# ronnymilleo/amcpy

Hardware: AMD Instinct MI355X
Metric: IQ frames/sec (18 features, 2048-sample complex64) (higher is better)
Workload: dtype f32; 1 GPU; 6 mods x 26 SNR x 4096 frames x 2048 samples complex64 per GPU (BASELINE configs[1]), resident in HBM; one launch per step; frame_size=2048, kernel=amcx_features18_wave_kernel<2048>

## Files before the change

amcpy_amd/csrc/amcx.hip:

```cpp
#include "../../include/amcx.h"

#include <hip/hip_runtime.h>
#include <stdio.h>
#include <stdlib.h>
#include <string.h>
#include <chrono>
#include <new>

#include "amcx_block_kernel.h"
#include "amcx_stream_kernel.h"
#include "amcx_wave_kernel.h"
#include "amcx_quad_kernel.h"
#include "amcx_group_kernel.h"
#include "amcx_short_kernel.h"
#include "amcx_post_kernels.h"
#include "amcx_pack_kernel.h"
#include "amcx_upload.h"

namespace {

thread_local char g_hip_err[256] = "";

int hip_fail(hipError_t e, const char* what) {
  snprintf(g_hip_err, sizeof g_hip_err, "%s: %s", what, hipGetErrorString(e));
  return AMCX_EHIP;
}

#define AMCX_HIP(call)                                     \
  do {                                                     \
    hipError_t e_ = (call);                                \
    if (e_ != hipSuccess) return hip_fail(e_, #call);      \
  } while (0)

bool is_pow2(int n) { return n > 0 && (n & (n - 1)) == 0; }

int resolve_variant(int32_t frame_size, int32_t variant) {
  if (frame_size < AMCX_MIN_FRAME_SIZE || frame_size > AMCX_MAX_FRAME_SIZE) return AMCX_EINVAL;
  const bool block_ok = frame_size <= AMCX_MAX_BLOCK_FRAME_SIZE;
  switch (variant) {
    case AMCX_VARIANT_AUTO:
      return amcx::wave_supports(frame_size) ? AMCX_VARIANT_WAVE : block_ok ? AMCX_VARIANT_BLOCK : AMCX_ENOTSUP;
    case AMCX_VARIANT_BLOCK:
      return block_ok ? AMCX_VARIANT_BLOCK : AMCX_ENOTSUP;
    case AMCX_VARIANT_WAVE:
      return amcx::wave_supports(frame_size) ? AMCX_VARIANT_WAVE : AMCX_ENOTSUP;
    default:
      return AMCX_EINVAL;
  }
}

int cu_count() {
  static int cus[64] = {};
  int dev = 0, n = 0;
  if (hipGetDevice(&dev) != hipSuccess) { (void)hipGetLastError(); return 256; }
  if (dev >= 0 && dev < 64 && cus[dev] > 0) return cus[dev];
  if (hipDeviceGetAttribute(&n, hipDeviceAttributeMultiprocessorCount, dev) != hipSuccess || n <= 0) {
    (void)hipGetLastError();
    return 256;
  }
  if (dev >= 0 && dev < 64) cus[dev] = n;
  return n;
}

bool on_another_device(const void* p) {
  hipPointerAttribute_t a;
  if (hipPointerGetAttributes(&a, p) != hipSuccess) { (void)hipGetLastError(); return false; }
  if (a.type != hipMemoryTypeDevice) return false;
  int dev = 0;
  if (hipGetDevice(&dev) != hipSuccess) { (void)hipGetLastError(); return false; }
  return a.device != dev;
}

int block_mode(int N) {
  if (is_pow2(N)) return amcx::kBlockPow2;
  if (N >= amcx::kBluesteinMinN && N <= amcx::kBluesteinMaxN) return amcx::kBlockBluestein;
  return N > amcx::kBluesteinMaxN ? amcx::kBlockBluesteinBig : amcx::kBlockDirect;
}

struct StreamPlan {
  int M;
  bool chirped;
  int64_t grid;
};

StreamPlan stream_plan(int32_t N, int64_t n_frames) {
  StreamPlan p;
  p.M = amcx::stream::conv_length(N);
  p.chirped = !is_pow2(N);
  p.grid = cu_count();
  if (p.grid > n_frames) p.grid = n_frames;
  if (p.grid < 1) p.grid = 1;
  return p;
}

int set_stream_lds_once(const void* kern, int which) {
  static bool attr_set[3][64] = {};
  int dev = 0;
  AMCX_HIP(hipGetDevice(&dev));
  if (dev < 0 || dev >= 64 || !attr_set[which][dev]) {
    const size_t most = which == 0 ? amcx::stream::lds_bytes(amcx::stream::kMaxN)
                        : which == 1 ? amcx::stream::lds_bytes_fft(amcx::stream::kMaxN)
                                     : (size_t)amcx::stream::kTileBytes + amcx::stream::kFftTabBytes;
    AMCX_HIP(hipFuncSetAttribute(kern, hipFuncAttributeMaxDynamicSharedMemorySize, (int)most));
    if (dev >= 0 && dev < 64) attr_set[which][dev] = true;
  }
  return AMCX_OK;
}

int launch_stream(const float2* iq, int64_t n_frames, int32_t N, int64_t row_stride, float* out,
                  int64_t out_stride, hipStream_t stream, void* ws, int64_t ws_bytes) {
  StreamPlan p = stream_plan(N, n_frames);
  const int64_t per = (int64_t)p.M * (int64_t)sizeof(float2);
  int64_t fit = ws != nullptr && ws_bytes > 0 ? ws_bytes / per - (p.chirped ? 1 : 0) : 0;
  if (fit >= 1 && (reinterpret_cast<uintptr_t>(ws) & 7u) == 0) {
    if (p.grid > fit) p.grid = fit;
    float2* const base = static_cast<float2*>(ws);
    const float2* bspec = nullptr;
    float2* bufs = base;
    if (p.chirped) {
      auto chirp = amcx::stream::amcx_stream_chirp_kernel;
      const int rc = set_stream_lds_once(reinterpret_cast<const void*>(chirp), 2);
      if (rc != AMCX_OK) return rc;
      hipLaunchKernelGGL(chirp, dim3(1), dim3(amcx::stream::kThreads),
                         (size_t)amcx::stream::kTileBytes + amcx::stream::kFftTabBytes, stream, base, (int)N, p.M);
      AMCX_HIP(hipGetLastError());
      bspec = base;
      bufs = base + p.M;
    }
    auto kern = amcx::stream::amcx_features18_stream_kernel<true>;
    const int rc = set_stream_lds_once(reinterpret_cast<const void*>(kern), 1);
    if (rc != AMCX_OK) return rc;
    hipLaunchKernelGGL(kern, dim3((unsigned)p.grid), dim3(amcx::stream::kThreads), amcx::stream::lds_bytes_fft(N), stream,
                       iq, (long long)n_frames, (int)N, (long long)row_stride, out, (long long)out_stride, bspec, bufs, p.M);
    AMCX_HIP(hipGetLastError());
    return AMCX_OK;
  }
  auto kern = amcx::stream::amcx_features18_stream_kernel<false>;
  const int rc = set_stream_lds_once(reinterpret_cast<const void*>(kern), 0);
  if (rc != AMCX_OK) return rc;
  hipLaunchKernelGGL(kern, dim3((unsigned)p.grid), dim3(amcx::stream::kThreads), amcx::stream::lds_bytes(N), stream, iq,
                     (long long)n_frames, (int)N, (long long)row_stride, out, (long long)out_stride,
                     static_cast<const float2*>(nullptr), static_cast<float2*>(nullptr), 0);
  AMCX_HIP(hipGetLastError());
  return AMCX_OK;
}

int launch_block(const float2* iq, int64_t n_frames, int32_t N, int64_t row_stride, float* out,
                 int64_t out_stride, hipStream_t stream, void* ws = nullptr, int64_t ws_bytes = 0) {
  if (N > amcx::kBlockMaxN) return launch_stream(iq, n_frames, N, row_stride, out, out_stride, stream, ws, ws_bytes);
  const int mode = block_mode(N);
  const size_t lds = (mode == amcx::kBlockBluestein      ? (size_t)16 * amcx::bluestein_length(N)
                      : mode == amcx::kBlockBluesteinBig ? (size_t)8 * amcx::kBluesteinBigM
                                                         : (size_t)16 * N) +
                     amcx::kBlockScratchBytes + amcx::kBlockTwiddleBytes;
  auto kern = mode == amcx::kBlockPow2           ? amcx::amcx_features18_block_kernel<amcx::kBlockPow2>
              : mode == amcx::kBlockBluestein    ? amcx::amcx_features18_block_kernel<amcx::kBlockBluestein>
              : mode == amcx::kBlockBluesteinBig ? amcx::amcx_features18_block_kernel<amcx::kBlockBluesteinBig>
                                                 : amcx::amcx_features18_block_kernel<amcx::kBlockDirect>;
  {
    static bool attr_set[4][64] = {};
    constexpr int kMaxLds = 16 * amcx::kBlockMaxN + amcx::kBlockScratchBytes + amcx::kBlockTwiddleBytes;
    int dev = 0;
    AMCX_HIP(hipGetDevice(&dev));
    if (dev < 0 || dev >= 64 || !attr_set[mode][dev]) {
      AMCX_HIP(hipFuncSetAttribute(reinterpret_cast<const void*>(kern),
                                   hipFuncAttributeMaxDynamicSharedMemorySize, kMaxLds));
      if (dev >= 0 && dev < 64) attr_set[mode][dev] = true;
    }
  }
  const int per_cu = (int)((160 * 1024) / lds) < 1 ? 1 : (int)((160 * 1024) / lds);
  int64_t grid = (int64_t)cu_count() * (per_cu > 8 ? 8 : per_cu) * 4;
  if (grid > n_frames) grid = n_frames;
  hipLaunchKernelGGL(kern, dim3((unsigned)grid), dim3(amcx::kBlockThreads), lds, stream, iq,
                     (long long)n_frames, (int)N, (long long)row_stride, out, (long long)out_stride);
  AMCX_HIP(hipGetLastError());
  return AMCX_OK;
}

__global__ __launch_bounds__(1024) void amcx_probe_fma_kernel(int iters, float* sink, unsigned long long* ticks) {
  float a0 = (float)threadIdx.x, a1 = a0 + 1.f, a2 = a0 + 2.f, a3 = a0 + 3.f, a4 = a0 + 4.f, a5 = a0 + 5.f,
        a6 = a0 + 6.f, a7 = a0 + 7.f;
  const float b0 = 1.0001f, b1 = 0.9999f;
  const unsigned long long t0 = __builtin_amdgcn_s_memtime();
  const unsigned long long r0 = __builtin_amdgcn_s_memrealtime();
  for (int i = 0; i < iters; ++i) {
#pragma unroll
    for (int u = 0; u < 4; ++u)
      asm volatile(
          "v_fma_f32 %0, %0, %8, %9\n v_fma_f32 %1, %1, %8, %9\n v_fma_f32 %2, %2, %8, %9\n v_fma_f32 %3, %3, %8, %9\n"
          "v_fma_f32 %4, %4, %8, %9\n v_fma_f32 %5, %5, %8, %9\n v_fma_f32 %6, %6, %8, %9\n v_fma_f32 %7, %7, %8, %9\n"
          : "+v"(a0), "+v"(a1), "+v"(a2), "+v"(a3), "+v"(a4), "+v"(a5), "+v"(a6), "+v"(a7) : "v"(b0), "v"(b1));
  }
  const unsigned long long t1 = __builtin_amdgcn_s_memtime();
  const unsigned long long r1 = __builtin_amdgcn_s_memrealtime();
  const float s = ((a0 + a1) + (a2 + a3)) + ((a4 + a5) + (a6 + a7));
  if (s == 12345.678f) sink[0] = s;
  if ((threadIdx.x & 63) == 0) {
    const long long w = ((long long)blockIdx.x * blockDim.x + threadIdx.x) >> 6;
    ticks[2 * w] = t1 - t0;
    ticks[2 * w + 1] = r1 - r0;
  }
}

__global__ __launch_bounds__(256) void amcx_probe_read_kernel(const float4* __restrict__ src,
                                                             long long n_vec, float* partial) {
  typedef float v4f __attribute__((ext_vector_type(4)));
  float acc = 0.f;
  const long long stride = (long long)gridDim.x * blockDim.x;
  long long i = (long long)blockIdx.x * blockDim.x + threadIdx.x;
  for (; i + 3 * stride < n_vec; i += 4 * stride) {
    const v4f a = __builtin_nontemporal_load(reinterpret_cast<const v4f*>(src + i));
    const v4f b = __builtin_nontemporal_load(reinterpret_cast<const v4f*>(src + i + stride));
    const v4f c = __builtin_nontemporal_load(reinterpret_cast<const v4f*>(src + i + 2 * stride));
    const v4f d = __builtin_nontemporal_load(reinterpret_cast<const v4f*>(src + i + 3 * stride));
    acc += ((a.x + a.y) + (a.z + a.w)) + ((b.x + b.y) + (b.z + b.w)) + ((c.x + c.y) + (c.z + c.w)) +
           ((d.x + d.y) + (d.z + d.w));
  }
  for (; i < n_vec; i += stride) {
    const float4 v = src[i];
    acc += (v.x + v.y) + (v.z + v.w);
  }
#pragma unroll
  for (int off = 32; off >= 1; off >>= 1) acc += __shfl_xor(acc, off, 64);
  __shared__ float s[4];
  if ((threadIdx.x & 63) == 0) s[threadIdx.x >> 6] = acc;
  __syncthreads();
  if (threadIdx.x == 0) partial[blockIdx.x] = (s[0] + s[1]) + (s[2] + s[3]);
}

}

extern "C" {

int amcx_abi_version(void) { return AMCX_ABI_VERSION; }

const char* amcx_strerror(int code) {
  switch (code) {
    case AMCX_OK: return "ok";
    case AMCX_EINVAL: return "invalid argument (null pointer, negative count, stride or frame_size out of range)";
    case AMCX_ENOTSUP: return "kernel variant does not support this frame_size";
    case AMCX_EHIP: return "HIP runtime error (see amcx_last_hip_error)";
    case AMCX_ENODEV: return "no usable gfx950 device";
    case AMCX_ENOMEM: return "device memory allocation failed";
    case AMCX_EIO: return "reading the container's file failed (see amcx_last_hip_error for the errno text)";
    default: return "unknown amcx error code";
  }
}

const char* amcx_last_hip_error(void) { return g_hip_err; }

int amcx_device_count(void) {
  int n = 0;
  hipError_t e = hipGetDeviceCount(&n);
  if (e == hipErrorNoDevice) return 0;
  if (e != hipSuccess) return hip_fail(e, "hipGetDeviceCount");
  int ok = 0;
  for (int d = 0; d < n; ++d) {
    hipDeviceProp_t p;
    if (hipGetDeviceProperties(&p, d) == hipSuccess && strncmp(p.gcnArchName, "gfx950", 6) == 0) ++ok;
  }
  return ok;
}

int64_t amcx_features18_workspace_bytes(int32_t frame_size, int64_t n_frames, int32_t variant) {
  if (n_frames < 0) return -1;
  const int v = resolve_variant(frame_size, variant);
  if (v < 0) return -1;
  if (v != AMCX_VARIANT_BLOCK || frame_size <= amcx::kBlockMaxN || n_frames == 0) return 0;
  const StreamPlan p = stream_plan(frame_size, n_frames);
  return (p.grid + (p.chirped ? 1 : 0)) * (int64_t)p.M * (int64_t)sizeof(float2);
}

int amcx_features18_c64_ws(const void* iq_dev, int64_t n_frames, int32_t frame_size,
                           int64_t row_stride_elems, float* out_dev, int64_t out_row_stride,
                           void* hip_stream, int32_t variant, void* workspace_dev, int64_t workspace_bytes) {
  if (n_frames < 0 || row_stride_elems < frame_size || out_row_stride < AMCX_NUM_FEATURES)
    return AMCX_EINVAL;
  const int v = resolve_variant(frame_size, variant);
  if (v < 0) return v;
  if (n_frames == 0) return AMCX_OK;
  if (iq_dev == nullptr || out_dev == nullptr) return AMCX_EINVAL;
  if ((reinterpret_cast<uintptr_t>(iq_dev) & 7u) || (reinterpret_cast<uintptr_t>(out_dev) & 3u))
    return AMCX_EINVAL;
  if (on_another_device(iq_dev) || on_another_device(out_dev)) return AMCX_EINVAL;
  hipStream_t stream = static_cast<hipStream_t>(hip_stream);
  const float2* iq = static_cast<const float2*>(iq_dev);
  if (v == AMCX_VARIANT_WAVE) {
    hipError_t e;
    if (frame_size == amcx::quad::kN)
      e = amcx::quad::launch_quad(iq, n_frames, row_stride_elems, out_dev, out_row_stride, stream, cu_count());
    else if (frame_size == amcx::group::G<8>::kN)
      e = amcx::group::launch_group<8>(iq, n_frames, row_stride_elems, out_dev, out_row_stride, stream, cu_count());
    else if (frame_size == amcx::group::G<16>::kN)
      e = amcx::group::launch_group<16>(iq, n_frames, row_stride_elems, out_dev, out_row_stride, stream, cu_count());
    else if (amcx::shortk::short_supports(frame_size))
      e = amcx::shortk::launch_short(iq, n_frames, frame_size, row_stride_elems, out_dev, out_row_stride, stream, cu_count());
    else
      e = amcx::launch_wave(iq, n_frames, frame_size, row_stride_elems, out_dev, out_row_stride, stream, cu_count());
    if (e != hipSuccess) return hip_fail(e, "wave kernel launch");
    return AMCX_OK;
  }
  if (workspace_dev != nullptr && on_another_device(workspace_dev)) return AMCX_EINVAL;
  return launch_block(iq, n_frames, frame_size, row_stride_elems, out_dev, out_row_stride, stream, workspace_dev,
                      workspace_bytes < 0 ? 0 : workspace_bytes);
}

int amcx_features18_c64_ex(const void* iq_dev, int64_t n_frames, int32_t frame_size,
                           int64_t row_stride_elems, float* out_dev, int64_t out_row_stride,
                           void* hip_stream, int32_t variant) {
  const int64_t want = n_frames > 0 && iq_dev != nullptr && out_dev != nullptr && row_stride_elems >= frame_size &&
                               out_row_stride >= AMCX_NUM_FEATURES
                           ? amcx_features18_workspace_bytes(frame_size, n_frames, variant) : 0;
  if (want <= 0)
    return amcx_features18_c64_ws(iq_dev, n_frames, frame_size, row_stride_elems, out_dev, out_row_stride, hip_stream,
                                  variant, nullptr, 0);
  hipStream_t st = static_cast<hipStream_t>(hip_stream);
  hipStreamCaptureStatus cap = hipStreamCaptureStatusNone;
  if (hipStreamIsCapturing(st, &cap) != hipSuccess) { (void)hipGetLastError(); cap = hipStreamCaptureStatusNone; }
  void* ws = nullptr;
  if (cap == hipStreamCaptureStatusNone && hipMallocAsync(&ws, (size_t)want, st) != hipSuccess) {
    (void)hipGetLastError();
    ws = nullptr;
  }
  if (ws == nullptr) {
    static const bool verbose = [] { const char* t = getenv("AMCX_VERBOSE"); return t != nullptr && t[0] != '\0' && t[0] != '0'; }();
    static std::atomic<bool> said{false};
    if (verbose && !said.exchange(true))
      fprintf(stderr, "amcx: frame_size %d runs the DFT by its definition (O(N^2)): %s; amcx_features18_c64_ws with %lld "
                      "bytes of workspace selects the FFT form\n", (int)frame_size,
              cap != hipStreamCaptureStatusNone ? "the stream is being captured" : "hipMallocAsync had no workspace", (long long)want);
  }
  const int rc = amcx_features18_c64_ws(iq_dev, n_frames, frame_size, row_stride_elems, out_dev, out_row_stride,
                                        hip_stream, variant, ws, ws != nullptr ? want : 0);
  if (ws != nullptr) {
    const hipError_t fe = hipFreeAsync(ws, st);
    if (rc == AMCX_OK) AMCX_HIP(fe);
  }
  return rc;
}

int amcx_features18_c64(const void* iq_dev, int64_t n_frames, int32_t frame_size,
                        int64_t row_stride_elems, float* out_dev, int64_t out_row_stride,
                        void* hip_stream) {
  return amcx_features18_c64_ex(iq_dev, n_frames, frame_size, row_stride_elems, out_dev,
                                out_row_stride, hip_stream, AMCX_VARIANT_AUTO);
}

}

namespace {

bool valid_feature_mask(uint32_t mask) { return mask != 0 && (mask & ~(uint32_t)AMCX_FEATURES_ALL) == 0; }

int subset_plan(int32_t N, int v, uint32_t mask) {
  if ((mask & 1u) != 0 || v != AMCX_VARIANT_WAVE) return amcx::kPlanAll;
  if (!amcx::shortk::short_supports(N) && N != 1024 && N != 2048 && N != 4096) return amcx::kPlanAll;
  return (mask & ~amcx::kMaskCumulants) == 0 ? amcx::kPlanCumulants : amcx::kPlanNoSpectral;
}

}

extern "C" {

int amcx_features_c64_subset(const void* iq_dev, int64_t n_frames, int32_t frame_size, int64_t row_stride_elems,
                             float* out_dev, int64_t out_row_stride, void* hip_stream, int32_t variant, uint32_t feature_mask,
                             void* workspace_dev, int64_t workspace_bytes) {
  if (!valid_feature_mask(feature_mask)) return AMCX_EINVAL;
  if (n_frames < 0 || row_stride_elems < frame_size || out_row_stride < AMCX_NUM_FEATURES) return AMCX_EINVAL;
  const int v = resolve_variant(frame_size, variant);
  if (v < 0) return v;
  if (n_frames == 0) return AMCX_OK;
  if (iq_dev == nullptr || out_dev == nullptr) return AMCX_EINVAL;
  hipStream_t stream = static_cast<hipStream_t>(hip_stream);
  const int plan = subset_plan(frame_size, v, feature_mask);
  if (plan == amcx::kPlanAll) {
    const int rc = amcx_features18_c64_ws(iq_dev, n_frames, frame_size, row_stride_elems, out_dev, out_row_stride,
                                          hip_stream, variant, workspace_dev, workspace_bytes);
    if (rc != AMCX_OK || feature_mask == (uint32_t)AMCX_FEATURES_ALL) return rc;
    int64_t grid = (n_frames * AMCX_NUM_FEATURES + 255) / 256;
    if (grid > 8192) grid = 8192;
    hipLaunchKernelGGL(amcx::amcx_mask_columns_kernel, dim3((unsigned)grid), dim3(256), 0, stream, out_dev, (long long)n_frames,
                       (long long)out_row_stride, (unsigned)feature_mask);
    AMCX_HIP(hipGetLastError());
    return AMCX_OK;
  }
  if ((reinterpret_cast<uintptr_t>(iq_dev) & 7u) || (reinterpret_cast<uintptr_t>(out_dev) & 3u)) return AMCX_EINVAL;
  if (on_another_device(iq_dev) || on_another_device(out_dev)) return AMCX_EINVAL;
  const float2* iq = static_cast<const float2*>(iq_dev);
  const bool short_n = amcx::shortk::short_supports(frame_size);
  hipError_t e;
  if (plan == amcx::kPlanCumulants)
    e = short_n ? amcx::shortk::launch_short_subset<amcx::kPlanCumulants>(iq, n_frames, frame_size, row_stride_elems, out_dev,
                                                                         out_row_stride, stream, cu_count(), feature_mask)
                : amcx::launch_wave_subset<amcx::kPlanCumulants>(iq, n_frames, frame_size, row_stride_elems, out_dev,
                                                                 out_row_stride, stream, cu_count(), feature_mask);
  else
    e = short_n ? amcx::shortk::launch_short_subset<amcx::kPlanNoSpectral>(iq, n_frames, frame_size, row_stride_elems, out_dev,
                                                                          out_row_stride, stream, cu_count(), feature_mask)
                : amcx::launch_wave_subset<amcx::kPlanNoSpectral>(iq, n_frames, frame_size, row_stride_elems, out_dev,
                                                                  out_row_stride, stream, cu_count(), feature_mask);
  if (e != hipSuccess) return hip_fail(e, "feature-subset kernel launch");
  return AMCX_OK;
}

struct amcx_ctx {
  int device = 0;
  hipStream_t stream = nullptr;
  float* d_out = nullptr; size_t out_cap = 0;
  amcx::Pool pool;
  int threads = 0;
  size_t slot_bytes = size_t(32) << 20;
  bool round_on_device = false;
  hipStream_t copy_stream = nullptr;
  char* pin = nullptr;     size_t pin_cap = 0;
  void* d_slab = nullptr;  size_t slab_cap = 0;
  void* d_frames = nullptr; size_t frames_cap = 0;
  void* d_ws = nullptr; size_t ws_cap = 0;
  hipEvent_t up_done[3] = {nullptr, nullptr, nullptr};
  hipEvent_t slab_free[2] = {nullptr, nullptr};
  float* out_pin = nullptr; size_t out_pin_cap = 0;
  amcx_upload_stats stats = {};
  char pci_bus_id[32] = {0};
  int numa_node = -1;
  std::vector<int> bind_cpus;
  struct SmallGraph {
    hipGraphExec_t exec = nullptr;
    int64_t frames = 0; int32_t frame_size = 0, variant = 0; bool c128 = false, zero_copy = false;
    const void* pin = nullptr; const void* slab = nullptr; const void* out = nullptr; const void* out_pin = nullptr;
    const void* ws = nullptr;
    size_t slot = 0;
    uint32_t mask = AMCX_FEATURES_ALL;
  };
  SmallGraph graphs[4];
  int graph_next = 0;
  int graph_hits = 0, graph_misses = 0;
  bool graphs_ok = true;
  std::atomic<int> in_call{0};
  std::atomic<uint32_t> feature_mask{AMCX_FEATURES_ALL};
};

}

namespace {

int ctx_reserve(void** p, size_t* cap, size_t bytes) {
  if (*cap >= bytes) return AMCX_OK;
  if (*p) { (void)hipFree(*p); *p = nullptr; *cap = 0; }
  size_t want = bytes < (size_t(1) << 20) ? bytes : bytes + bytes / 4;
  if (hipMalloc(p, want) != hipSuccess) {
    (void)hipGetLastError();
    if (want == bytes || hipMalloc(p, bytes) != hipSuccess) { (void)hipGetLastError(); *p = nullptr; return AMCX_ENOMEM; }
    want = bytes;
  }
  *cap = want;
  return AMCX_OK;
}

void ctx_reserve_ws(amcx_ctx* c, int32_t N, int64_t frames, int32_t variant) {
  const int64_t want = amcx_features18_workspace_bytes(N, frames, variant);
  if (want > 0 && ctx_reserve(&c->d_ws, &c->ws_cap, (size_t)want) != AMCX_OK) { c->d_ws = nullptr; c->ws_cap = 0; }
}

int ctx_features(amcx_ctx* c, const void* rows, int64_t frames, int32_t N, float* out, int32_t variant, uint32_t mask) {
  const int64_t want = amcx_features18_workspace_bytes(N, frames, variant);
  const bool have = want > 0 && c->d_ws != nullptr && c->ws_cap >= (size_t)want;
  if (mask != (uint32_t)AMCX_FEATURES_ALL)
    return amcx_features_c64_subset(rows, frames, N, N, out, AMCX_NUM_FEATURES, c->stream, variant, mask,
                                    have ? c->d_ws : nullptr, have ? want : 0);
  return amcx_features18_c64_ws(rows, frames, N, N, out, AMCX_NUM_FEATURES, c->stream, variant, have ? c->d_ws : nullptr,
                                have ? want : 0);
}

struct DeviceGuard {
  int prev = -1;
  hipError_t enter(int dev) {
    hipError_t e = hipGetDevice(&prev);
    if (e != hipSuccess) { prev = -1; return e; }
    return hipSetDevice(dev);
  }
  ~DeviceGuard() { if (prev >= 0) (void)hipSetDevice(prev); }
};

constexpr int kPinSlots = 3;

using amcx::classify_layout;

double wall_now() {
  return std::chrono::duration<double>(std::chrono::steady_clock::now().time_since_epoch()).count();
}

int strided_prepare(amcx_ctx* c, size_t slot, size_t dslot, size_t frames_bytes, size_t out_bytes, bool threaded) {
  if (c->threads == 0) {
    unsigned hw = std::thread::hardware_concurrency();
    if (!c->bind_cpus.empty()) hw = (unsigned)amcx::allowed_subset(c->bind_cpus).size();
    c->threads = (int)(hw == 0 ? 4 : hw > 8 ? 8 : hw);
  }
  if (threaded) c->pool.resize(c->threads);
  if (c->copy_stream == nullptr) AMCX_HIP(hipStreamCreateWithFlags(&c->copy_stream, hipStreamNonBlocking));
  for (auto& ev : c->up_done) if (ev == nullptr) AMCX_HIP(hipEventCreateWithFlags(&ev, hipEventDisableTiming));
  for (auto& ev : c->slab_free) if (ev == nullptr) AMCX_HIP(hipEventCreateWithFlags(&ev, hipEventDisableTiming));
  if (c->pin_cap < kPinSlots * slot) {
    if (c->pin) { (void)hipHostFree(c->pin); c->pin = nullptr; c->pin_cap = 0; }
    if (hipHostMalloc(reinterpret_cast<void**>(&c->pin), kPinSlots * slot, hipHostMallocDefault) != hipSuccess) {
      (void)hipGetLastError();
      c->pin = nullptr;
      return AMCX_ENOMEM;
    }
    c->pin_cap = kPinSlots * slot;
  }
  if (c->out_pin_cap < out_bytes) {
    if (c->out_pin) { (void)hipHostFree(c->out_pin); c->out_pin = nullptr; c->out_pin_cap = 0; }
    const size_t want = out_bytes + out_bytes / 4 + 4096;
    if (hipHostMalloc(reinterpret_cast<void**>(&c->out_pin), want, hipHostMallocDefault) != hipSuccess) {
      (void)hipGetLastError();
      c->out_pin = nullptr;
      return AMCX_ENOMEM;
    }
    c->out_pin_cap = want;
  }
  int rc = ctx_reserve(&c->d_slab, &c->slab_cap, 2 * dslot);
  if (rc == AMCX_OK && frames_bytes) rc = ctx_reserve(&c->d_frames, &c->frames_cap, frames_bytes);
  if (rc == AMCX_OK) rc = ctx_reserve(reinterpret_cast<void**>(&c->d_out), &c->out_cap, out_bytes);
  return rc;
}

int ctx_run_strided(amcx_ctx* c, amcx::Source src, int64_t S, int64_t K,
                    int32_t N, int64_t ss, int64_t sk, int64_t sn, float* out_host, int64_t out_row_stride,
                    int32_t variant) {
  if (c == nullptr) return AMCX_EINVAL;
  const int32_t kind = src.kind;
  if (S < 0 || K < 0 || ss < 0 || sk < 0 || sn < 0 || out_row_stride < AMCX_NUM_FEATURES ||
      kind < AMCX_SRC_C64 || kind > AMCX_SRC_F64_SPLIT)
    return AMCX_EINVAL;
  const int v = resolve_variant(N, variant);
  if (v < 0) return v;
  if (S == 0 || K == 0) return AMCX_OK;
  if (S > (int64_t(1) << 40) / K) return AMCX_EINVAL;
  if ((src.fd < 0 && src.re == nullptr) || (src.fd >= 0 && src.re_off < 0) || out_host == nullptr) return AMCX_EINVAL;
  struct InCall {
    std::atomic<int>& n;
    explicit InCall(std::atomic<int>& c) : n(c) { n.fetch_add(1, std::memory_order_acq_rel); }
    ~InCall() { n.fetch_sub(1, std::memory_order_acq_rel); }
  } in_call(c->in_call);
  const uint32_t mask = c->feature_mask.load(std::memory_order_acquire);
  if (kind < AMCX_SRC_F32_SPLIT) { src.im = nullptr; src.im_off = -1; }
  std::atomic<int> io_error{0};
  src.io_error = &io_error;
  const int64_t F = S * K;
  bool rows = false, inner_snr = false;
  amcx::RunMap map;
  if (!classify_layout(S, K, N, ss, sk, sn, &rows, &inner_snr, &map)) return AMCX_ENOTSUP;
  if (!rows && S > 0x7fffffffLL) return AMCX_EINVAL;
  const bool as_c128 = c->round_on_device && kind == AMCX_SRC_C128;
  const size_t esz = as_c128 ? 16 : 8;
  const size_t src_esz = kind == AMCX_SRC_C64 ? 8 : kind == AMCX_SRC_C128 ? 16 : kind == AMCX_SRC_F32_SPLIT ? 4 : 8;
  const int64_t unit = rows ? N : F;
  const int64_t n_units = rows ? F : N;
  size_t slot = c->slot_bytes;
  const size_t total_staged = (size_t)unit * esz * (size_t)n_units;
  if (slot > total_staged) slot = total_staged;
  if (slot < (size_t)unit * esz) slot = (size_t)unit * esz;
  if (slot > (size_t(4) << 30)) return AMCX_ENOMEM;
  slot = (slot + 4095) & ~size_t(4095);

  DeviceGuard guard;
  AMCX_HIP(guard.enter(c->device));
  const double t_start = wall_now();
  const size_t dslot = (rows && as_c128) ? slot + slot / 2 : slot;
  const bool threaded = total_staged >= (size_t(1) << 20);
  static const std::vector<int> kNoCpus;
  amcx::AffinityGuard on_local_cpus(threaded ? c->bind_cpus : kNoCpus);
  int rc = strided_prepare(c, slot, dslot, rows ? 0 : (size_t)F * N * 8, sizeof(float) * AMCX_NUM_FEATURES * (size_t)F,
                           threaded);
  if (rc != AMCX_OK) return rc;
  ctx_reserve_ws(c, N, F, v);
  amcx::Pool inline_pool;
  amcx_upload_stats st = {};
  amcx::Pool& pool = threaded ? c->pool : inline_pool;
  st.frames = F; st.threads = pool.size(); st.plane_major = rows ? 0 : 1; st.from_file = src.fd >= 0 ? 1 : 0;
  st.source_bytes = F * (int64_t)N * (int64_t)src_esz * ((kind >= AMCX_SRC_F32_SPLIT && src.has_im()) ? 2 : 1);

  hipError_t e = hipSuccess;
  const double t_loop = wall_now();
  if (rows && !threaded && total_staged <= slot && c->graphs_ok && getenv("AMCX_NO_GRAPH") == nullptr) {
    char* pinned = c->pin;
    char* dev = static_cast<char*>(c->d_slab);
    const size_t bytes = (size_t)n_units * (size_t)unit * esz;
    const size_t out_bytes = sizeof(float) * AMCX_NUM_FEATURES * (size_t)F;
    double t0 = wall_now();
    amcx::stage_runs(inline_pool, pinned, src, map, 0, n_units, as_c128);
    st.seconds_staging += wall_now() - t0;
    if (io_error.load() != 0) {
      snprintf(g_hip_err, sizeof g_hip_err, "reading the container's file: %s", strerror(io_error.load()));
      return AMCX_EIO;
    }
    const bool zero_copy = !as_c128 && bytes <= (size_t(64) << 10) && getenv("AMCX_NO_ZERO_COPY") == nullptr;
    amcx_ctx::SmallGraph* g = nullptr;
    for (auto& cand : c->graphs)
      if (cand.exec && cand.frames == F && cand.frame_size == N && cand.variant == v && cand.c128 == as_c128 &&
          cand.zero_copy == zero_copy &&
          cand.pin == pinned && cand.slab == dev && cand.out == c->d_out && cand.out_pin == c->out_pin && cand.slot == slot &&
          cand.ws == c->d_ws && cand.mask == mask)
        g = &cand;
    if (g != nullptr) {
      ++c->graph_hits;
    } else {
      ++c->graph_misses;
      if (c->graph_misses > 64 && c->graph_misses > 4 * c->graph_hits) c->graphs_ok = false;
      amcx_ctx::SmallGraph& slot_g = c->graphs[c->graph_next];
      hipGraph_t graph = nullptr;
      hipGraphExec_t exec = nullptr;
      int crc = AMCX_OK;
      hipError_t ce = hipStreamBeginCapture(c->stream, hipStreamCaptureModeThreadLocal);
      if (ce == hipSuccess && zero_copy) {
        crc = ctx_features(c, pinned, F, N, c->out_pin, v, mask);
        const hipError_t ee = hipStreamEndCapture(c->stream, &graph);
        ce = ee;
      } else if (ce == hipSuccess) {
        ce = hipMemcpyAsync(dev, pinned, bytes, hipMemcpyHostToDevice, c->stream);
        const void* d_rows = dev;
        if (ce == hipSuccess && as_c128) {
          float2* rounded = reinterpret_cast<float2*>(dev + slot);
          hipLaunchKernelGGL(amcx::amcx_c128_to_c64_kernel, dim3(2048), dim3(256), 0, c->stream,
                             reinterpret_cast<const double2*>(dev), (long long)F, (int)N, (long long)N, rounded);
          ce = hipGetLastError();
          d_rows = rounded;
        }
        if (ce == hipSuccess) crc = ctx_features(c, d_rows, F, N, c->d_out, v, mask);
        if (ce == hipSuccess && crc == AMCX_OK)
          ce = hipMemcpyAsync(c->out_pin, c->d_out, out_bytes, hipMemcpyDeviceToHost, c->stream);
        const hipError_t ee = hipStreamEndCapture(c->stream, &graph);
        if (ce == hipSuccess) ce = ee;
      }
      if (ce == hipSuccess && crc == AMCX_OK && graph != nullptr) ce = hipGraphInstantiate(&exec, graph, nullptr, nullptr, 0);
      if (graph != nullptr) (void)hipGraphDestroy(graph);
      if (ce != hipSuccess || crc != AMCX_OK || exec == nullptr) {
        (void)hipGetLastError();
        c->graphs_ok = false;
      } else {
        if (slot_g.exec) (void)hipGraphExecDestroy(slot_g.exec);
        slot_g.exec = exec; slot_g.frames = F; slot_g.frame_size = N; slot_g.variant = v; slot_g.c128 = as_c128;
        slot_g.zero_copy = zero_copy;
        slot_g.pin = pinned; slot_g.slab = dev; slot_g.out = c->d_out; slot_g.out_pin = c->out_pin; slot_g.slot = slot;
        slot_g.ws = c->d_ws;
        slot_g.mask = mask;
        c->graph_next = (c->graph_next + 1) % 4;
        g = &slot_g;
      }
    }
    if (g != nullptr) {
      st.seconds_prepare = t_loop - t_start;
      const double t_tail = wall_now();
      e = hipGraphLaunch(g->exec, c->stream);
      const hipError_t e2 = hipStreamSynchronize(c->stream);
      if (e != hipSuccess || e2 != hipSuccess) return hip_fail(e != hipSuccess ? e : e2, "amcx_ctx_features18 (graph launch)");
      if (out_row_stride == AMCX_NUM_FEATURES) {
        memcpy(out_host, c->out_pin, out_bytes);
      } else {
        for (int64_t gi = 0; gi < F; ++gi)
          memcpy(out_host + (size_t)gi * (size_t)out_row_stride, c->out_pin + (size_t)gi * AMCX_NUM_FEATURES,
                 sizeof(float) * AMCX_NUM_FEATURES);
      }
      st.pcie_bytes = (int64_t)bytes; st.chunks = 1;
      st.seconds_tail = wall_now() - t_tail;
      st.seconds = wall_now() - t_start;
      c->stats = st;
      return AMCX_OK;
    }
  }
  const int64_t units_per_slot = (int64_t)(slot / ((size_t)unit * esz));
  int64_t u = 0;
  for (int ch = 0; u < n_units && rc == AMCX_OK; ++ch) {
    int64_t take = units_per_slot;
    if (ch < 12) {
      const int64_t ramp = (int64_t)((size_t(2) << 20 << (ch / 2)) / ((size_t)unit * esz));
      if (ramp < take) take = ramp;
    }
    if (take < 1) take = 1;
    if (take > n_units - u) take = n_units - u;
    const int ps = ch % kPinSlots, ds = ch & 1;
    char* pinned = c->pin + (size_t)ps * slot;
    char* dev = static_cast<char*>(c->d_slab) + (size_t)ds * dslot;
    const size_t bytes = (size_t)take * (size_t)unit * esz;
    if (ch >= kPinSlots) {
      const double t0 = wall_now();
      e = hipEventSynchronize(c->up_done[ps]);
      st.seconds_waiting += wall_now() - t0;
      if (e != hipSuccess) break;
    }
    {
      const double t0 = wall_now();
      const int64_t per_unit = rows ? 1 : map.cnt_b;
      amcx::stage_runs(pool, pinned, src, map, u * per_unit, (u + take) * per_unit, as_c128);
      st.seconds_staging += wall_now() - t0;
      if (io_error.load() != 0) {
        snprintf(g_hip_err, sizeof g_hip_err, "reading the container's file: %s", strerror(io_error.load()));
        rc = AMCX_EIO;
        break;
      }
    }
    if (ch >= 2) { e = hipStreamWaitEvent(c->copy_stream, c->slab_free[ds], 0); if (e != hipSuccess) break; }
    e = hipMemcpyAsync(dev, pinned, bytes, hipMemcpyHostToDevice, c->copy_stream);
    if (e != hipSuccess) break;
    e = hipEventRecord(c->up_done[ps], c->copy_stream);
    if (e != hipSuccess) break;
    e = hipStreamWaitEvent(c->stream, c->up_done[ps], 0);
    if (e != hipSuccess) break;
    st.pcie_bytes += (int64_t)bytes;
    if (rows) {
      const void* d_rows = dev;
      if (as_c128) {
        float2* rounded = reinterpret_cast<float2*>(dev + slot);
        hipLaunchKernelGGL(amcx::amcx_c128_to_c64_kernel, dim3(2048), dim3(256), 0, c->stream,
                           reinterpret_cast<const double2*>(dev), (long long)take, (int)N, (long long)N, rounded);
        e = hipGetLastError();
        if (e != hipSuccess) break;
        d_rows = rounded;
      }
      rc = ctx_features(c, d_rows, take, N, c->d_out + (size_t)u * AMCX_NUM_FEATURES, v, mask);
    } else {
      float2* frames = static_cast<float2*>(c->d_frames);
      e = as_c128 ? amcx::launch_pack_planes(reinterpret_cast<const double2*>(dev), (int)take, (long long)F, (long long)F,
                                             (int)S, (long long)K, inner_snr ? 1 : 0, frames, (long long)N, (int)u, c->stream)
                  : amcx::launch_pack_planes(reinterpret_cast<const float2*>(dev), (int)take, (long long)F, (long long)F,
                                             (int)S, (long long)K, inner_snr ? 1 : 0, frames, (long long)N, (int)u, c->stream);
      if (e != hipSuccess) break;
    }
    if (rc != AMCX_OK) break;
    e = hipEventRecord(c->slab_free[ds], c->stream);
    if (e != hipSuccess) break;
    u += take;
    st.chunks = ch + 1;
  }
  if (rc == AMCX_OK && e == hipSuccess && !rows)
    rc = ctx_features(c, c->d_frames, F, N, c->d_out, v, mask);
  const double t_tail = wall_now();
  st.seconds_prepare = t_loop - t_start;
  if (rc == AMCX_OK && e == hipSuccess)
    e = hipMemcpyAsync(c->out_pin, c->d_out, sizeof(float) * AMCX_NUM_FEATURES * (size_t)F, hipMemcpyDeviceToHost, c->stream);
  if (rc == AMCX_OK && e != hipSuccess) rc = hip_fail(e, "amcx_ctx_features18_strided_host");
  hipError_t e2 = hipStreamSynchronize(c->stream);
  hipError_t e1 = (rc == AMCX_OK && e2 == hipSuccess) ? hipSuccess : hipStreamSynchronize(c->copy_stream);
  if (rc == AMCX_OK && (e1 != hipSuccess || e2 != hipSuccess))
    rc = hip_fail(e1 != hipSuccess ? e1 : e2, "amcx_ctx_features18_strided_host (sync)");
  if (rc == AMCX_OK) {
    if (out_row_stride == AMCX_NUM_FEATURES) {
      memcpy(out_host, c->out_pin, sizeof(float) * AMCX_NUM_FEATURES * (size_t)F);
    } else {
      for (int64_t g = 0; g < F; ++g)
        memcpy(out_host + (size_t)g * (size_t)out_row_stride, c->out_pin + (size_t)g * AMCX_NUM_FEATURES,
               sizeof(float) * AMCX_NUM_FEATURES);
    }
  }
  st.seconds_tail = wall_now() - t_tail;
  st.seconds = wall_now() - t_start;
  c->stats = st;
  return rc;
}

int ctx_run(amcx_ctx* c, const void* iq_host, bool is_c128, int64_t n_frames, int32_t frame_size,
            int64_t row_stride_elems, float* out_host, int64_t out_row_stride, int32_t variant) {
  if (c == nullptr) return AMCX_EINVAL;
  if (n_frames < 0 || row_stride_elems < frame_size || out_row_stride < AMCX_NUM_FEATURES) return AMCX_EINVAL;
  amcx::Source src;
  src.re = static_cast<const char*>(iq_host);
  src.kind = is_c128 ? AMCX_SRC_C128 : AMCX_SRC_C64;
  return ctx_run_strided(c, src, 1, n_frames, frame_size, 0, row_stride_elems, 1, out_host, out_row_stride, variant);
}

}

extern "C" {

int amcx_ctx_create(int32_t device, amcx_ctx** ctx_out) {
  if (ctx_out == nullptr) return AMCX_EINVAL;
  *ctx_out = nullptr;
  int ndev = 0;
  if (hipGetDeviceCount(&ndev) != hipSuccess || ndev <= 0 || device < 0 || device >= ndev) {
    (void)hipGetLastError();
    return AMCX_ENODEV;
  }
  DeviceGuard guard;
  AMCX_HIP(guard.enter(device));
  amcx_ctx* c = new (std::nothrow) amcx_ctx();
  if (c == nullptr) return AMCX_ENOMEM;
  c->device = device;
  hipError_t e = hipStreamCreateWithFlags(&c->stream, hipStreamNonBlocking);
  if (e != hipSuccess) { delete c; return hip_fail(e, "hipStreamCreateWithFlags"); }
  {
    void* warm_pin = nullptr;
    void* warm_dev = nullptr;
    if (hipHostMalloc(&warm_pin, 4096, hipHostMallocDefault) == hipSuccess && hipMalloc(&warm_dev, 4096) == hipSuccess) {
      memset(warm_pin, 0, 4096);
      if (hipMemcpyAsync(warm_dev, warm_pin, 4096, hipMemcpyHostToDevice, c->stream) == hipSuccess)
        (void)hipStreamSynchronize(c->stream);
    }
    if (warm_dev != nullptr) (void)hipFree(warm_dev);
    if (warm_pin != nullptr) (void)hipHostFree(warm_pin);
    (void)hipGetLastError();
  }
  if (hipDeviceGetPCIBusId(c->pci_bus_id, (int)sizeof c->pci_bus_id, device) != hipSuccess) {
    (void)hipGetLastError();
    c->pci_bus_id[0] = '\0';
  }
  const char* numa_env = getenv("AMCX_NUMA");
  if (c->pci_bus_id[0] != '\0' && !(numa_env != nullptr && numa_env[0] == '0')) {
    const char* root = getenv("AMCX_SYSFS_ROOT");
    const amcx::NumaPlace place = amcx::numa_place_of(root != nullptr && root[0] != '\0' ? root : "/sys", c->pci_bus_id);
    if (!place.empty()) {
      c->numa_node = place.node;
      c->bind_cpus = place.cpus;
      c->pool.set_cpus(c->bind_cpus);
    }
  }
  *ctx_out = c;
  return AMCX_OK;
}

int amcx_ctx_bind_cpus(amcx_ctx* ctx, const int32_t* cpus, int32_t n_cpus) {
  if (ctx == nullptr || n_cpus < 0 || (n_cpus > 0 && cpus == nullptr)) return AMCX_EINVAL;
  std::vector<int> v;
  for (int32_t i = 0; i < n_cpus; ++i) {
    if (cpus[i] < 0 || cpus[i] >= CPU_SETSIZE) return AMCX_EINVAL;
    v.push_back((int)cpus[i]);
  }
  if (ctx->in_call.load(std::memory_order_acquire) != 0) return AMCX_EINVAL;
  ctx->bind_cpus = v;
  if (v.empty()) ctx->numa_node = -1;
  ctx->pool.set_cpus(ctx->bind_cpus);
  return AMCX_OK;
}

int amcx_ctx_set_feature_mask(amcx_ctx* ctx, uint32_t feature_mask) {
  if (ctx == nullptr || !valid_feature_mask(feature_mask)) return AMCX_EINVAL;
  int idle = 0;
  if (!ctx->in_call.compare_exchange_strong(idle, 1, std::memory_order_acq_rel)) return AMCX_EINVAL;
  ctx->feature_mask.store(feature_mask, std::memory_order_release);
  ctx->in_call.fetch_sub(1, std::memory_order_acq_rel);
  return AMCX_OK;
}

int amcx_ctx_placement(const amcx_ctx* ctx, amcx_placement* out) {
  if (ctx == nullptr || out == nullptr) return AMCX_EINVAL;
  memset(out, 0, sizeof *out);
  out->device = ctx->device;
  out->numa_node = ctx->numa_node;
  out->n_cpus = (int32_t)ctx->bind_cpus.size();
  out->n_cpus_allowed = (int32_t)amcx::allowed_subset(ctx->bind_cpus).size();
  out->first_cpu = ctx->bind_cpus.empty() ? -1 : ctx->bind_cpus.front();
  out->last_cpu = ctx->bind_cpus.empty() ? -1 : ctx->bind_cpus.back();
  snprintf(out->pci_bus_id, sizeof out->pci_bus_id, "%s", ctx->pci_bus_id);
  return AMCX_OK;
}

int amcx_device_pci_bus_id(int32_t device, char* buf, int32_t buf_len) {
  if (buf == nullptr || buf_len < 16) return AMCX_EINVAL;
  buf[0] = '\0';
  int ndev = 0;
  if (hipGetDeviceCount(&ndev) != hipSuccess || ndev <= 0 || device < 0 || device >= ndev) {
    (void)hipGetLastError();
    return AMCX_ENODEV;
  }
  AMCX_HIP(hipDeviceGetPCIBusId(buf, buf_len, device));
  for (char* p = buf; *p; ++p) *p = (char)tolower((unsigned char)*p);
  return AMCX_OK;
}

int amcx_numa_place(const char* sysfs_root, const char* pci_bus_id, int32_t* node_out, int32_t* cpus_out,
                    int32_t cpus_cap, int32_t* n_cpus_out) {
  if (pci_bus_id == nullptr || node_out == nullptr || n_cpus_out == nullptr || cpus_cap < 0 ||
      (cpus_cap > 0 && cpus_out == nullptr))
    return AMCX_EINVAL;
  const amcx::NumaPlace place = amcx::numa_place_of(sysfs_root != nullptr && sysfs_root[0] != '\0' ? sysfs_root : "/sys", pci_bus_id);
  *node_out = place.empty() ? -1 : place.node;
  *n_cpus_out = place.empty() ? 0 : (int32_t)place.cpus.size();
  for (int32_t i = 0; i < *n_cpus_out && i < cpus_cap; ++i) cpus_out[i] = place.cpus[(size_t)i];
  return AMCX_OK;
}

int amcx_ctx_destroy(amcx_ctx* c) {
  if (c == nullptr) return AMCX_OK;
  DeviceGuard guard;
  (void)guard.enter(c->device);
  if (c->stream) { (void)hipStreamSynchronize(c->stream); (void)hipStreamDestroy(c->stream); }
  if (c->copy_stream) { (void)hipStreamSynchronize(c->copy_stream); (void)hipStreamDestroy(c->copy_stream); }
  for (auto ev : c->up_done) if (ev) (void)hipEventDestroy(ev);
  for (auto ev : c->slab_free) if (ev) (void)hipEventDestroy(ev);
  if (c->d_out) (void)hipFree(c->d_out);
  if (c->d_slab) (void)hipFree(c->d_slab);
  if (c->d_frames) (void)hipFree(c->d_frames);
  if (c->d_ws) (void)hipFree(c->d_ws);
  if (c->pin) (void)hipHostFree(c->pin);
  if (c->out_pin) (void)hipHostFree(c->out_pin);
  for (auto& g : c->graphs) if (g.exec) (void)hipGraphExecDestroy(g.exec);
  delete c;
  return AMCX_OK;
}

int amcx_ctx_features18_strided_host(amcx_ctx* ctx, const void* re, const void* im, int32_t kind,
                                     int64_t n_snr, int64_t n_frames, int32_t frame_size,
                                     int64_t stride_snr, int64_t stride_frame, int64_t stride_sample,
                                     float* out_host, int64_t out_row_stride, int32_t variant) {
  amcx::Source src;
  src.re = static_cast<const char*>(re);
  src.im = static_cast<const char*>(im);
  src.kind = kind;
  return ctx_run_strided(ctx, src, n_snr, n_frames, frame_size, stride_snr, stride_frame, stride_sample,
                         out_host, out_row_stride, variant);
}

int amcx_ctx_features18_strided_file(amcx_ctx* ctx, int32_t fd, int64_t re_offset, int64_t im_offset, int32_t kind,
                                     int64_t n_snr, int64_t n_frames, int32_t frame_size,
                                     int64_t stride_snr, int64_t stride_frame, int64_t stride_sample,
                                     float* out_host, int64_t out_row_stride, int32_t variant) {
  if (fd < 0 || re_offset < 0) return AMCX_EINVAL;
  amcx::Source src;
  src.fd = fd;
  src.re_off = re_offset;
  src.im_off = im_offset;
  src.kind = kind;
  return ctx_run_strided(ctx, src, n_snr, n_frames, frame_size, stride_snr, stride_frame, stride_sample,
                         out_host, out_row_stride, variant);
}

static int stage_any(amcx::Source src, int64_t n_snr, int64_t n_frames,
                     int32_t frame_size, int64_t stride_snr, int64_t stride_frame, int64_t stride_sample,
                     int64_t first_unit, int64_t n_units, void* dst, int64_t dst_bytes, int32_t threads,
                     int32_t* plane_major, int32_t* inner_snr_out) {
  const int32_t kind = src.kind;
  if (n_snr < 0 || n_frames < 0 || stride_snr < 0 || stride_frame < 0 || stride_sample < 0 || first_unit < 0 ||
      n_units < 0 || threads < 0 || threads > 256 || kind < AMCX_SRC_C64 || kind > AMCX_SRC_F64_SPLIT ||
      frame_size < AMCX_MIN_FRAME_SIZE || frame_size > AMCX_MAX_FRAME_SIZE)
    return AMCX_EINVAL;
  if (n_frames > 0 && n_snr > (int64_t(1) << 40) / n_frames) return AMCX_EINVAL;
  bool rows = false, inner_snr = false;
  amcx::RunMap map;
  if (!classify_layout(n_snr, n_frames, frame_size, stride_snr, stride_frame, stride_sample, &rows, &inner_snr, &map))
    return AMCX_ENOTSUP;
  if (plane_major) *plane_major = rows ? 0 : 1;
  if (inner_snr_out) *inner_snr_out = inner_snr ? 1 : 0;
  const int64_t F = n_snr * n_frames, unit = rows ? frame_size : F, total_units = rows ? F : frame_size;
  if (first_unit + n_units > total_units) return AMCX_EINVAL;
  if (n_units == 0 || unit == 0) return AMCX_OK;
  if ((src.fd < 0 && src.re == nullptr) || dst == nullptr || dst_bytes < n_units * unit * 8) return AMCX_EINVAL;
  if (kind < AMCX_SRC_F32_SPLIT) { src.im = nullptr; src.im_off = -1; }
  std::atomic<int> io_error{0};
  src.io_error = &io_error;
  amcx::Pool pool;
  pool.resize(threads < 1 ? 1 : threads);
  const int64_t per_unit = rows ? 1 : map.cnt_b;
  amcx::stage_runs(pool, static_cast<char*>(dst), src, map, first_unit * per_unit, (first_unit + n_units) * per_unit, false);
  if (io_error.load() != 0) {
    snprintf(g_hip_err, sizeof g_hip_err, "reading the container's file: %s", strerror(io_error.load()));
    return AMCX_EIO;
  }
  return AMCX_OK;
}

int amcx_stage_host(const void* re, const void* im, int32_t kind, int64_t n_snr, int64_t n_frames,
                    int32_t frame_size, int64_t stride_snr, int64_t stride_frame, int64_t stride_sample,
                    int64_t first_unit, int64_t n_units, void* dst, int64_t dst_bytes, int32_t threads,
                    int32_t* plane_major, int32_t* inner_snr_out) {
  amcx::Source src;
  src.re = static_cast<const char*>(re);
  src.im = static_cast<const char*>(im);
  src.kind = kind;
  return stage_any(src, n_snr, n_frames, frame_size, stride_snr, stride_frame, stride_sample, first_unit, n_units, dst,
                   dst_bytes, threads, plane_major, inner_snr_out);
}

int amcx_stage_file(int32_t fd, int64_t re_offset, int64_t im_offset, int32_t kind, int64_t n_snr, int64_t n_frames,
                    int32_t frame_size, int64_t stride_snr, int64_t stride_frame, int64_t stride_sample,
                    int64_t first_unit, int64_t n_units, void* dst, int64_t dst_bytes, int32_t threads,
                    int32_t* plane_major, int32_t* inner_snr_out) {
  if (fd < 0 || re_offset < 0) return AMCX_EINVAL;
  amcx::Source src;
  src.fd = fd;
  src.re_off = re_offset;
  src.im_off = im_offset;
  src.kind = kind;
  return stage_any(src, n_snr, n_frames, frame_size, stride_snr, stride_frame, stride_sample, first_unit, n_units, dst,
                   dst_bytes, threads, plane_major, inner_snr_out);
}

int amcx_ctx_configure(amcx_ctx* ctx, int32_t threads, int64_t slot_bytes, int32_t round_on_device) {
  if (ctx == nullptr || threads < 0 || threads > 256 || slot_bytes < 0) return AMCX_EINVAL;
  if (threads > 0) ctx->threads = threads;
  if (slot_bytes > 0) ctx->slot_bytes = (size_t)slot_bytes < 4096 ? 4096 : (size_t)slot_bytes;
  if (round_on_device >= 0) ctx->round_on_device = round_on_device != 0;
  return AMCX_OK;
}

int amcx_ctx_upload_stats(const amcx_ctx* ctx, amcx_upload_stats* out) {
  if (ctx == nullptr || out == nullptr) return AMCX_EINVAL;
  *out = ctx->stats;
  return AMCX_OK;
}

int amcx_pack_planes_c64(const void* slab_dev, int32_t src_kind, int32_t n_planes, int64_t plane_stride,
                         int64_t n_snr, int64_t n_frames, int32_t inner_snr, void* frames_dev,
                         int64_t row_stride_elems, int32_t n0, void* hip_stream) {
  if (n_planes < 0 || n_snr < 0 || n_frames < 0 || n0 < 0 || (src_kind != AMCX_SRC_C64 && src_kind != AMCX_SRC_C128))
    return AMCX_EINVAL;
  if (n_snr > 0x7fffffffLL || (n_frames > 0 && n_snr > (int64_t(1) << 40) / n_frames)) return AMCX_EINVAL;
  const int64_t P = n_snr * n_frames;
  if (plane_stride < P || row_stride_elems < (int64_t)n0 + n_planes) return AMCX_EINVAL;
  if (n_planes == 0 || P == 0) return AMCX_OK;
  if (slab_dev == nullptr || frames_dev == nullptr) return AMCX_EINVAL;
  if (on_another_device(slab_dev) || on_another_device(frames_dev)) return AMCX_EINVAL;
  hipStream_t stream = static_cast<hipStream_t>(hip_stream);
  float2* dst = static_cast<float2*>(frames_dev);
  hipError_t e = src_kind == AMCX_SRC_C128
      ? amcx::launch_pack_planes(static_cast<const double2*>(slab_dev), n_planes, P, plane_stride, (int)n_snr, n_frames,
                                 inner_snr, dst, row_stride_elems, n0, stream)
      : amcx::launch_pack_planes(static_cast<const float2*>(slab_dev), n_planes, P, plane_stride, (int)n_snr, n_frames,
                                 inner_snr, dst, row_stride_elems, n0, stream);
  if (e != hipSuccess) return hip_fail(e, "amcx_pack_planes_c64");
  return AMCX_OK;
}

int amcx_ctx_features18_c64_host(amcx_ctx* ctx, const void* iq_host, int64_t n_frames, int32_t frame_size,
                                 int64_t row_stride_elems, float* out_host, int64_t out_row_stride,
                                 int32_t variant) {
  return ctx_run(ctx, iq_host, false, n_frames, frame_size, row_stride_elems, out_host, out_row_stride, variant);
}

int amcx_ctx_features18_c128_host(amcx_ctx* ctx, const void* iq_host, int64_t n_frames, int32_t frame_size,
                                  int64_t row_stride_elems, float* out_host, int64_t out_row_stride,
                                  int32_t variant) {
  return ctx_run(ctx, iq_host, true, n_frames, frame_size, row_stride_elems, out_host, out_row_stride, variant);
}

static int one_shot(const void* iq_host, bool is_c128, int64_t n_frames, int32_t frame_size,
                    int64_t row_stride_elems, float* out_host, int64_t out_row_stride, int32_t device,
                    int32_t variant) {
  if (n_frames < 0 || row_stride_elems < frame_size || out_row_stride < AMCX_NUM_FEATURES)
    return AMCX_EINVAL;
  const int v = resolve_variant(frame_size, variant);
  if (v < 0) return v;
  if (n_frames == 0) return AMCX_OK;
  if (iq_host == nullptr || out_host == nullptr) return AMCX_EINVAL;
  amcx_ctx* c = nullptr;
  int rc = amcx_ctx_create(device, &c);
  if (rc != AMCX_OK) return rc;
  rc = ctx_run(c, iq_host, is_c128, n_frames, frame_size, row_stride_elems, out_host, out_row_stride, v);
  (void)amcx_ctx_destroy(c);
  return rc;
}

int amcx_features18_c64_host(const void* iq_host, int64_t n_frames, int32_t frame_size,
                             int64_t row_stride_elems, float* out_host, int64_t out_row_stride,
                             int32_t device, int32_t variant) {
  return one_shot(iq_host, false, n_frames, frame_size, row_stride_elems, out_host, out_row_stride, device, variant);
}

int amcx_features18_c128_host(const void* iq_host, int64_t n_frames, int32_t frame_size,
                              int64_t row_stride_elems, float* out_host, int64_t out_row_stride,
                              int32_t device, int32_t variant) {
  return one_shot(iq_host, true, n_frames, frame_size, row_stride_elems, out_host, out_row_stride, device, variant);
}

int amcx_kernel_name(int32_t frame_size, int32_t variant, char* buf, int32_t buf_len) {
  if (buf == nullptr || buf_len <= 0) return AMCX_EINVAL;
  const int v = resolve_variant(frame_size, variant);
  if (v < 0) return v;
  const char* name = (v == AMCX_VARIANT_WAVE) ? amcx::wave_kernel_name(frame_size)
                     : frame_size > amcx::kBlockMaxN                   ? "amcx_features18_stream_kernel"
                     : block_mode(frame_size) == amcx::kBlockPow2      ? "amcx_features18_block_kernel<1>"
                     : block_mode(frame_size) == amcx::kBlockBluestein ? "amcx_features18_block_kernel<2>"
                     : block_mode(frame_size) == amcx::kBlockBluesteinBig ? "amcx_features18_block_kernel<3>"
                                                                       : "amcx_features18_block_kernel<0>";
  snprintf(buf, (size_t)buf_len, "%s", name);
  return AMCX_OK;
}

int amcx_kernel_name_subset(int32_t frame_size, int32_t variant, uint32_t feature_mask, char* buf, int32_t buf_len) {
  if (buf == nullptr || buf_len <= 0 || !valid_feature_mask(feature_mask)) return AMCX_EINVAL;
  const int v = resolve_variant(frame_size, variant);
  if (v < 0) return v;
  const int plan = subset_plan(frame_size, v, feature_mask);
  if (plan == amcx::kPlanAll) return amcx_kernel_name(frame_size, variant, buf, buf_len);
  snprintf(buf, (size_t)buf_len, "%s<%d, %d>",
           amcx::shortk::short_supports(frame_size) ? "amcx_features_subset_short_kernel" : "amcx_features_subset_wave_kernel",
           (int)frame_size, plan);
  return AMCX_OK;
}

int amcx_probe_fma_rate(double seconds, void* hip_stream, double* wave_instr_per_s, double* clock_ghz) {
  if (!(seconds > 0.0) || seconds > 60.0 || wave_instr_per_s == nullptr) return AMCX_EINVAL;
  *wave_instr_per_s = 0.0;
  if (clock_ghz) *clock_ghz = 0.0;
  hipStream_t stream = static_cast<hipStream_t>(hip_stream);
  const int grid = cu_count();
  if (grid <= 0) return AMCX_ENODEV;
  const long long n_waves = (long long)grid * 16;
  constexpr int kIters = 32768;
  float* sink = nullptr;
  unsigned long long* ticks = nullptr;
  hipEvent_t e0 = nullptr, e1 = nullptr, e2 = nullptr;
  int rc = AMCX_OK;
  auto fail = [&](hipError_t e, const char* what) { rc = hip_fail(e, what); };
  hipError_t e = hipMalloc(reinterpret_cast<void**>(&sink), 4);
  if (e == hipSuccess) e = hipMalloc(reinterpret_cast<void**>(&ticks), (size_t)n_waves * 16);
  if (e == hipSuccess) e = hipEventCreate(&e0);
  if (e == hipSuccess) e = hipEventCreate(&e1);
  if (e == hipSuccess) e = hipEventCreate(&e2);
  if (e != hipSuccess) {
    fail(e, "fma probe setup");
  } else {
    auto launch = [&]() { hipLaunchKernelGGL(amcx_probe_fma_kernel, dim3((unsigned)grid), dim3(1024), 0, stream, kIters, sink, ticks); };
    (void)hipEventRecord(e0, stream);
    launch();
    (void)hipEventRecord(e1, stream);
    e = hipEventSynchronize(e1);
    float one_ms = 0.f;
    if (e == hipSuccess) e = hipEventElapsedTime(&one_ms, e0, e1);
    if (e != hipSuccess) {
      fail(e, "fma probe launch");
    } else {
      if (!(one_ms > 0.01f)) one_ms = 0.01f;
      long long n = (long long)(seconds * 1e3 / 2.0 / one_ms);
      if (n < 1) n = 1;
      if (n > 100000) n = 100000;
      for (long long i = 0; i < n; ++i) launch();
      (void)hipEventRecord(e1, stream);
      for (long long i = 0; i < n; ++i) launch();
      (void)hipEventRecord(e2, stream);
      e = hipEventSynchronize(e2);
      float ms = 0.f;
      if (e == hipSuccess) e = hipEventElapsedTime(&ms, e1, e2);
      if (e == hipSuccess) e = hipGetLastError();
      if (e != hipSuccess || !(ms > 0.f)) {
        fail(e, "fma probe timing");
      } else {
        *wave_instr_per_s = (double)n * (double)n_waves * (double)kIters * 32.0 / ((double)ms * 1e-3);
        if (clock_ghz) {
          std::vector<unsigned long long> h((size_t)n_waves * 2);
          e = hipMemcpy(h.data(), ticks, h.size() * 8, hipMemcpyDeviceToHost);
          if (e == hipSuccess) {
            double cyc = 0.0, real = 0.0;
            for (long long w = 0; w < n_waves; ++w) { cyc += (double)h[(size_t)(2 * w)]; real += (double)h[(size_t)(2 * w + 1)]; }
            if (real > 0.0) *clock_ghz = cyc / (real * 10.0);
          } else {
            fail(e, "fma probe read-back");
          }
        }
      }
    }
  }
  if (e0) (void)hipEventDestroy(e0);
  if (e1) (void)hipEventDestroy(e1);
  if (e2) (void)hipEventDestroy(e2);
  if (sink) (void)hipFree(sink);
  if (ticks) (void)hipFree(ticks);
  return rc;
}

int amcx_probe_read_bw(const void* src_dev, int64_t n_bytes, float* partial_dev, void* hip_stream) {
  if (src_dev == nullptr || partial_dev == nullptr || n_bytes < 0 || (n_bytes & 15)) return AMCX_EINVAL;
  if (n_bytes == 0) return AMCX_OK;
  hipLaunchKernelGGL(amcx_probe_read_kernel, dim3(4096), dim3(256), 0,
                     static_cast<hipStream_t>(hip_stream), static_cast<const float4*>(src_dev),
                     (long long)(n_bytes / 16), partial_dev);
  AMCX_HIP(hipGetLastError());
  return AMCX_OK;
}

static void stats_plan(int64_t n_groups, int64_t rows_per_group, int n_cols, int64_t* chunks, int64_t* rows_per_chunk) {
  const int64_t tile = amcx::stat_tile_rows(n_cols);
  const int64_t tiles = (rows_per_group + tile - 1) / tile;
  const int64_t target = 1024;
  int64_t want = (target + n_groups - 1) / n_groups;
  if (want > tiles) want = tiles;
  if (want < 1) want = 1;
  const int64_t tiles_per_chunk = (tiles + want - 1) / want;
  *rows_per_chunk = tiles_per_chunk * tile;
  *chunks = (tiles + tiles_per_chunk - 1) / tiles_per_chunk;
}

static bool stats_args_ok(int64_t n_groups, int64_t rows_per_group, int64_t row_stride, int32_t n_cols) {
  return n_groups >= 0 && rows_per_group >= 1 && n_cols >= 1 && n_cols <= amcx::kStatMaxCols &&
         row_stride >= n_cols && row_stride <= (1 << 20) && n_groups <= 0x7fffffffLL;
}

int64_t amcx_group_stats_workspace_bytes(int64_t n_groups, int64_t rows_per_group, int32_t n_cols) {
  if (!stats_args_ok(n_groups, rows_per_group, n_cols, n_cols)) return -1;
  if (n_groups == 0) return 0;
  int64_t chunks, rpc;
  stats_plan(n_groups, rows_per_group, n_cols, &chunks, &rpc);
  return n_groups * chunks * n_cols * 3 * (int64_t)sizeof(double);
}

int amcx_group_stats_ws_f32(const float* x_dev, int64_t n_groups, int64_t rows_per_group,
                            int64_t row_stride, int32_t n_cols, double* mean_dev, double* std_dev,
                            void* workspace_dev, int64_t workspace_bytes, void* hip_stream) {
  if (!stats_args_ok(n_groups, rows_per_group, row_stride, n_cols)) return AMCX_EINVAL;
  if (n_groups == 0) return AMCX_OK;
  if (x_dev == nullptr || mean_dev == nullptr || std_dev == nullptr || workspace_dev == nullptr) return AMCX_EINVAL;
  if (on_another_device(x_dev) || on_another_device(workspace_dev)) return AMCX_EINVAL;
  int64_t chunks, rpc;
  stats_plan(n_groups, rows_per_group, n_cols, &chunks, &rpc);
  if (workspace_bytes < n_groups * chunks * n_cols * 3 * (int64_t)sizeof(double)) return AMCX_EINVAL;
  if (n_groups * chunks > 0x7fffffffLL) return AMCX_EINVAL;
  hipStream_t st = static_cast<hipStream_t>(hip_stream);
  double* part = static_cast<double*>(workspace_dev);
  hipLaunchKernelGGL(amcx::amcx_stats_part_kernel, dim3((unsigned)(n_groups * chunks)),
                     dim3(amcx::kStatThreads), 0, st, x_dev, (long long)rows_per_group,
                     (long long)row_stride, (int)n_cols, (long long)rpc, (int)chunks, part);
  const unsigned pool_threads = chunks > 128 ? 256u : chunks > 64 ? 128u : 64u;
  for (int64_t g0 = 0; g0 < n_groups; g0 += 65535) {
    const int64_t ng = n_groups - g0 < 65535 ? n_groups - g0 : 65535;
    hipLaunchKernelGGL(amcx::amcx_stats_combine_kernel, dim3((unsigned)n_cols, (unsigned)ng), dim3(pool_threads), 0, st,
                       part + g0 * n_cols * 3 * chunks, (int)chunks, (int)n_cols, mean_dev + g0 * n_cols,
                       std_dev + g0 * n_cols);
  }
  AMCX_HIP(hipGetLastError());
  return AMCX_OK;
}

int amcx_group_stats_f32(const float* x_dev, int64_t n_groups, int64_t rows_per_group,
                         int64_t row_stride, int32_t n_cols, double* mean_dev, double* std_dev,
                         void* hip_stream) {
  if (!stats_args_ok(n_groups, rows_per_group, row_stride, n_cols)) return AMCX_EINVAL;
  if (n_groups == 0) return AMCX_OK;
  if (x_dev == nullptr || mean_dev == nullptr || std_dev == nullptr) return AMCX_EINVAL;
  const int64_t bytes = amcx_group_stats_workspace_bytes(n_groups, rows_per_group, n_cols);
  hipStream_t st = static_cast<hipStream_t>(hip_stream);
  void* ws = nullptr;
  AMCX_HIP(hipMallocAsync(&ws, (size_t)bytes, st));
  const int rc = amcx_group_stats_ws_f32(x_dev, n_groups, rows_per_group, row_stride, n_cols, mean_dev,
                                         std_dev, ws, bytes, hip_stream);
  const hipError_t fe = hipFreeAsync(ws, st);
  if (rc != AMCX_OK) return rc;
  AMCX_HIP(fe);
  return AMCX_OK;
}

int64_t amcx_standardize_workspace_bytes(int64_t n_rows, int32_t n_cols) {
  if (n_rows < 1) return n_rows == 0 ? 0 : -1;
  const int64_t part = amcx_group_stats_workspace_bytes(1, n_rows, n_cols);
  return part < 0 ? -1 : part + 2 * (int64_t)amcx::kStatMaxCols * (int64_t)sizeof(double);
}

int amcx_standardize_fit_transform_f32(const float* x_dev, int64_t n_rows, int64_t row_stride,
                                       int32_t n_cols, const int32_t* cols_host, int32_t n_sel,
                                       float* out_dev, int64_t out_stride, double* mean_dev,
                                       double* scale_dev, void* workspace_dev, int64_t workspace_bytes,
                                       void* hip_stream) {
  if (n_rows < 0 || n_sel < 1 || n_sel > amcx::kStatMaxCols || out_stride < n_sel || cols_host == nullptr ||
      n_cols < 1 || n_cols > amcx::kStatMaxCols || row_stride < n_cols)
    return AMCX_EINVAL;
  amcx::SelectCols sel;
  sel.n = n_sel;
  for (int j = 0; j < amcx::kStatMaxCols; ++j) sel.c[j] = 0;
  for (int j = 0; j < n_sel; ++j) {
    if (cols_host[j] < 0 || cols_host[j] >= n_cols) return AMCX_EINVAL;
    sel.c[j] = cols_host[j];
  }
  if (n_rows == 0) return AMCX_OK;
  if (!x_dev || !out_dev || !mean_dev || !scale_dev || !workspace_dev) return AMCX_EINVAL;
  if (on_another_device(x_dev) || on_another_device(out_dev)) return AMCX_EINVAL;
  const int64_t need = amcx_standardize_workspace_bytes(n_rows, n_cols);
  if (need < 0 || workspace_bytes < need) return AMCX_EINVAL;
  double* all_mean = static_cast<double*>(workspace_dev);
  double* all_std = all_mean + amcx::kStatMaxCols;
  void* part = all_std + amcx::kStatMaxCols;
  const int rc = amcx_group_stats_ws_f32(x_dev, 1, n_rows, row_stride, n_cols, all_mean, all_std, part,
                                         need - 2 * (int64_t)amcx::kStatMaxCols * (int64_t)sizeof(double), hip_stream);
  if (rc != AMCX_OK) return rc;
  const int64_t grid = (n_rows + amcx::kSelectRows - 1) / amcx::kSelectRows;
  if (grid > 0x7fffffffLL) return AMCX_EINVAL;
  hipLaunchKernelGGL(amcx::amcx_select_fit_scale_kernel, dim3((unsigned)grid), dim3(amcx::kBlockThreads), 0,
                     static_cast<hipStream_t>(hip_stream), x_dev, (long long)n_rows, (long long)row_stride, sel,
                     all_mean, all_std, out_dev, (long long)out_stride, mean_dev, scale_dev);
  AMCX_HIP(hipGetLastError());
  return AMCX_OK;
}

int amcx_select_scale_f32(const float* x_dev, int64_t n_rows, int64_t row_stride,
                          const int32_t* cols_dev, int32_t n_sel, const double* mean_dev,
                          const double* scale_dev, float* out_dev, int64_t out_stride,
                          void* hip_stream) {
  if (n_rows < 0 || n_sel < 1 || out_stride < n_sel || row_stride < 1) return AMCX_EINVAL;
  if (n_rows == 0) return AMCX_OK;
  if (!x_dev || !cols_dev || !mean_dev || !scale_dev || !out_dev) return AMCX_EINVAL;
  const int64_t total = n_rows * n_sel;
  int64_t grid = (total + amcx::kBlockThreads - 1) / amcx::kBlockThreads;
  const int64_t cap = (int64_t)cu_count() * 8;
  if (grid > cap) grid = cap;
  hipLaunchKernelGGL(amcx::amcx_select_scale_kernel, dim3((unsigned)grid), dim3(amcx::kBlockThreads), 0,
                     static_cast<hipStream_t>(hip_stream), x_dev, (long long)n_rows, (long long)row_stride,
                     cols_dev, (int)n_sel, mean_dev, scale_dev, out_dev, (long long)out_stride);
  AMCX_HIP(hipGetLastError());
  return AMCX_OK;
}

}
```

amcpy_amd/csrc/amcx_wave_kernel.h:

```cpp
#pragma once

#include <type_traits>
#include <utility>

#include "amcx_math.h"

#ifndef AMCX_PRIO_MASK
#define AMCX_PRIO_MASK 7
#endif
#define AMCX_PRIO_OF(b) ((AMCX_PRIO_MASK >> (b)) & 1)

namespace amcx {

constexpr int kPlanAll = 0, kPlanNoSpectral = 1, kPlanCumulants = 2;
constexpr unsigned kMaskAll = 0x3FFFFu, kMaskCumulants = 0x3FE00u;
constexpr unsigned kMaskFreq = (1u << 4) | (1u << 8);
__device__ __forceinline__ void mask_columns(float (&feat)[18], unsigned mask) {
#pragma unroll
  for (int j = 0; j < 18; ++j)
    if (!((mask >> j) & 1u)) feat[j] = __builtin_nanf("");
}

namespace wave {

constexpr int kNumSums = 27;
constexpr int kStashStride = 33;

constexpr int kEx1StrideKK = 136, kEx1StrideB = 68;
constexpr int kEx2StrideK2 = 65;
constexpr int kExchangeBytes = (7 * kEx1StrideKK + kEx1StrideB + 64) * 8;
constexpr int kTw2Stride = 15 * 8;
constexpr int kTw3Row = 64 * 8;

template <int N>
struct Cfg {
  static_assert(N == 1024 || N == 2048 || N == 4096, "one wave per frame (128 ... 512: amcx_short_kernel.h; 8192 up: quad / group)");
  static constexpr bool kSplit = N == 4096;
  static constexpr int kFramesPerWave = N == 2048 ? 4 : 8;
  static constexpr int kFlushes = N == 4096 ? 2 : 1;
  static constexpr int kStashBytes = kFramesPerWave * kFlushes * kStashStride * 4;
  static constexpr int kTailChunk = 2;
  static constexpr int kRunFrames = kFramesPerWave;
  static constexpr int kWavesPerWG = kSplit ? 8 : 16;
  static constexpr int kThreads = 64 * kWavesPerWG;
  static constexpr int kTailFrames = kWavesPerWG * kFramesPerWave;
  static constexpr int kRows = N / 128;
  static constexpr int kHeldRows = kRows;
  static constexpr int kFftRows = kSplit ? 16 : kRows;
  static constexpr int kFftN = 128 * kFftRows;
  static constexpr int kPhases = kFftRows >= 8 ? kFftRows / 8 : 1;
  static constexpr int kT2Bytes = 8 * kPhases * kTw2Stride;
  static constexpr int kT3Bytes = kPhases * 2 * 7 * kTw3Row;
  static constexpr int kT4Bytes = kSplit ? 64 * 16 : 0;
  static constexpr int kTableBytes = kT2Bytes + kT3Bytes + kT4Bytes;
  static constexpr int kCounterOffset = kTableBytes + kWavesPerWG * (kExchangeBytes + kStashBytes);
  static constexpr int kLdsBytes = kCounterOffset + 16;
  static_assert(kLdsBytes <= 163840, "one workgroup per CU must fit in 160 KiB of LDS");
  static_assert(kFramesPerWave <= 64, "one frame per lane in the finaliser");
  static_assert(kSplit || 2 * kRows * 64 * 4 <= kExchangeBytes, "|x| parking must fit the exchange buffer");
};

template <int... I, class F>
__device__ __forceinline__ void static_for_impl(std::integer_sequence<int, I...>, F&& f) {
  (f(std::integral_constant<int, I>{}), ...);
}
template <int N, class F>
__device__ __forceinline__ void static_for(F&& f) {
  static_for_impl(std::make_integer_sequence<int, N>{}, static_cast<F&&>(f));
}

constexpr int bitrev(int v, int bits) {
  int r = 0;
  for (int i = 0; i < bits; ++i) r |= ((v >> i) & 1) << (bits - 1 - i);
  return r;
}

constexpr float kC32[16] = {1.f, 0.98078528040323043f, 0.92387953251128674f, 0.83146961230254524f,
                            0.70710678118654752f, 0.55557023301960218f, 0.38268343236508977f, 0.19509032201612825f,
                            0.f, -0.19509032201612825f, -0.38268343236508977f, -0.55557023301960218f,
                            -0.70710678118654752f, -0.83146961230254524f, -0.92387953251128674f, -0.98078528040323043f};
constexpr float kS32[16] = {0.f, 0.19509032201612825f, 0.38268343236508977f, 0.55557023301960218f,
                            0.70710678118654752f, 0.83146961230254524f, 0.92387953251128674f, 0.98078528040323043f,
                            1.f, 0.98078528040323043f, 0.92387953251128674f, 0.83146961230254524f,
                            0.70710678118654752f, 0.55557023301960218f, 0.38268343236508977f, 0.19509032201612825f};

template <int J>
__device__ __forceinline__ void mul_w32(float& r, float& i) {
  constexpr float h = 0.70710678118654752f;
  if constexpr (J == 0) {
  } else if constexpr (J == 8) {
    const float t = r; r = i; i = -t;
  } else if constexpr (J == 4) {
    const float t = (r + i) * h; i = (i - r) * h; r = t;
  } else if constexpr (J == 12) {
    const float t = (i - r) * h; i = (-r - i) * h; r = t;
  } else {
    constexpr float c = kC32[J], s = kS32[J];
    const float t = __builtin_fmaf(r, c, i * s);
    i = __builtin_fmaf(i, c, -(r * s));
    r = t;
  }
}

constexpr float kCosPi32[17] = {1.f, 0.99518472667219689f, 0.98078528040323043f, 0.95694033573220882f,
                                0.92387953251128674f, 0.88192126434835503f, 0.83146961230254524f,
                                0.77301045336273696f, 0.70710678118654752f, 0.63439328416364549f,
                                0.55557023301960218f, 0.47139673682599764f, 0.38268343236508977f,
                                0.29028467725446236f, 0.19509032201612825f, 0.09801714032956060f, 0.f};
template <int J>
__device__ __forceinline__ void mul_w64(float& r, float& i) {
  static_assert(J >= 0 && J < 32, "upper half-plane only");
  if constexpr (J % 2 == 0) {
    mul_w32<J / 2>(r, i);
  } else {
    constexpr float c = J <= 16 ? kCosPi32[J] : -kCosPi32[32 - J];
    constexpr float s = kCosPi32[J <= 16 ? 16 - J : J - 16];
    const float t = __builtin_fmaf(r, c, i * s);
    i = __builtin_fmaf(i, c, -(r * s));
    r = t;
  }
}

template <int LEN, int OFF, int R>
__device__ __forceinline__ void dif(float (&re)[R], float (&im)[R]) {
  if constexpr (LEN >= 2) {
    constexpr int H = LEN / 2;
    static_for<H>([&](auto jj) {
      constexpr int j = decltype(jj)::value;
      const float ar = re[OFF + j], ai = im[OFF + j], br = re[OFF + j + H], bi = im[OFF + j + H];
      re[OFF + j] = ar + br;
      im[OFF + j] = ai + bi;
      float dr = ar - br, di = ai - bi;
      mul_w32<j * (32 / LEN)>(dr, di);
      re[OFF + j + H] = dr;
      im[OFF + j + H] = di;
    });
    dif<H, OFF, R>(re, im);
    dif<H, OFF + H, R>(re, im);
  }
}

template <int LEN, int OFF, int R>
__device__ __forceinline__ void dif_stage(float (&re)[R], float (&im)[R]) {
  constexpr int H = LEN / 2;
  static_for<H>([&](auto jj) {
    constexpr int j = decltype(jj)::value;
    const float ar = re[OFF + j], ai = im[OFF + j], br = re[OFF + j + H], bi = im[OFF + j + H];
    re[OFF + j] = ar + br;
    im[OFF + j] = ai + bi;
    float dr = ar - br, di = ai - bi;
    mul_w32<j * (32 / LEN)>(dr, di);
    re[OFF + j + H] = dr;
    im[OFF + j + H] = di;
  });
}


template <int CTRL, int ROW_MASK = 0xf, int BANK_MASK = 0xf, bool BOUND = true>
__device__ __forceinline__ float dpp(float v) {
  return __builtin_bit_cast(float, __builtin_amdgcn_update_dpp(0, __builtin_bit_cast(int, v), CTRL,
                                                                ROW_MASK, BANK_MASK, BOUND));
}
constexpr int kQuadXor1 = 0xB1;
constexpr int kQuadXor2 = 0x4E;
constexpr int kRowHalfMirror = 0x141, kRowMirror = 0x140, kRowBcast15 = 0x142, kRowBcast31 = 0x143;
constexpr int kWaveRol1 = 0x134;

__device__ __forceinline__ float wave_sum_l63(float v) {
  v += dpp<kQuadXor1>(v);
  v += dpp<kQuadXor2>(v);
  v += dpp<kRowHalfMirror>(v);
  v += dpp<kRowMirror>(v);
  v += dpp<kRowBcast15, 0xa, 0xf, false>(v);
  v += dpp<kRowBcast31, 0xc, 0xf, false>(v);
  return v;
}
__device__ __forceinline__ float wave_max_l63(float v) {
  v = __builtin_fmaxf(v, dpp<kQuadXor1>(v));
  v = __builtin_fmaxf(v, dpp<kQuadXor2>(v));
  v = __builtin_fmaxf(v, dpp<kRowHalfMirror>(v));
  v = __builtin_fmaxf(v, dpp<kRowMirror>(v));
  v = __builtin_fmaxf(v, dpp<kRowBcast15, 0xa, 0xf, false>(v));
  v = __builtin_fmaxf(v, dpp<kRowBcast31, 0xc, 0xf, false>(v));
  return v;
}
__device__ __forceinline__ float bcast_l63(float v) {
  return __builtin_bit_cast(float, __builtin_amdgcn_readlane(__builtin_bit_cast(int, v), 63));
}

__device__ __forceinline__ void lds_wave_fence() {
  __builtin_amdgcn_fence(__ATOMIC_ACQ_REL, "wavefront");
  __builtin_amdgcn_wave_barrier();
}

#ifdef AMCX_WAVE_STAMPS
#define AMCX_STAMP_ARG , unsigned long long* __restrict__ stamp_out
#if AMCX_WAVE_STAMPS == 1
#define AMCX_STAMP(sec)                                                               \
  do {                                                                                \
    __builtin_amdgcn_sched_barrier(0);                                                \
    unsigned long long t_;                                                            \
    asm volatile("s_memtime %0\n\ts_waitcnt lgkmcnt(0)" : "=s"(t_)::"memory");        \
    __builtin_amdgcn_sched_barrier(0);                                                \
    stamp_acc[sec] += t_ - stamp_last;                                                \
    stamp_last = t_;                                                                  \
  } while (0)
#else
#define AMCX_STAMP(sec) do { } while (0)
#endif
#else
#define AMCX_STAMP_ARG
#define AMCX_STAMP(sec) do { } while (0)
#endif
constexpr int kStampSections = 8;

struct WaveLanes {
  static constexpr float kInvLanes = 1.0f / 64.0f;
  static __device__ __forceinline__ float sum_all(float v) { return bcast_l63(wave_sum_l63(v)); }
  static __device__ __forceinline__ float next_lane(float v) { return dpp<kWaveRol1>(v); }
  static __device__ __forceinline__ bool is_last(int lane) { return lane == 63; }
};

template <class Lanes>
struct StatsT {
  float sA = 0, sBh = 0, sP = 0, sAA = 0, sX4 = 0, sAB = 0, sAP = 0, sBP = 0;
  float sAAA = 0, sABB = 0, sAAB = 0, sBBB = 0, sAAP = 0, sX4P = 0, sABP = 0;
  float sa = 0, st1 = 0, st2 = 0, sab1 = 0, sab2 = 0, sw1 = 0, sw2 = 0, sw3 = 0, sw4 = 0;
  float sad1 = 0, sad2 = 0, sad4 = 0;
  float Kt = 0, Kw = 0, Ka = 0;
  float th_b1_prev = 0;
  float rot_prev = 0;
  float wmax = 0;

  __device__ __forceinline__ void step(float w) {
    const float d = w - Kw, d2 = d * d;
    sw1 += d; sw2 += d2;
    sw3 = __builtin_fmaf(d2, d, sw3);
    sw4 = __builtin_fmaf(d2, d2, sw4);
  }

  template <bool FIRST, bool LAST>
  __device__ __forceinline__ void row(float re0, float im0, float re1, float im1, int lane,
                                      float& a0, float& a1) {
    float th[2];
    const float res[2] = {re0, re1}, ims[2] = {im0, im1};
    float av[2];
    static_for<2>([&](auto bb) {
      constexpr int b = decltype(bb)::value;
      const float re = res[b], im = ims[b];
      const float q = __builtin_fmaf(im, im, kTinyPower);
      const float P = __builtin_fmaf(re, re, q);
      const float A = __builtin_fmaf(re, re, -q);
      const float Bh = re * im;
      const float AA = A * A, BB = Bh * Bh, AP = A * P;
      const float X4 = __builtin_fmaf(-4.0f, BB, AA);
      sA += A; sBh += Bh; sP += P; sAA += AA; sX4 += X4; sAP += AP;
      sAB = __builtin_fmaf(A, Bh, sAB);
      sBP = __builtin_fmaf(Bh, P, sBP);
      sAAA = __builtin_fmaf(AA, A, sAAA);
      sABB = __builtin_fmaf(A, BB, sABB);
      sAAB = __builtin_fmaf(AA, Bh, sAAB);
      sBBB = __builtin_fmaf(BB, Bh, sBBB);
      sAAP = __builtin_fmaf(AA, P, sAAP);
      sX4P = __builtin_fmaf(X4, P, sX4P);
      sABP = __builtin_fmaf(AP, Bh, sABP);
      av[b] = __builtin_amdgcn_sqrtf(P);
      sa += av[b];
      th[b] = fast_angle(re, im, av[b]);
    });
    a0 = av[0]; a1 = av[1];
    if constexpr (FIRST) {
      const float w00 = wrapped_step(th[1], th[0]);
      Kt = Lanes::sum_all(th[0]) * Lanes::kInvLanes;
      Kw = Lanes::sum_all(w00) * Lanes::kInvLanes;
      Ka = Lanes::sum_all(__builtin_fabsf(th[0])) * Lanes::kInvLanes;
    }
    static_for<2>([&](auto bb) {
      constexpr int b = decltype(bb)::value;
      const float d = th[b] - Kt;
      st1 += d;
      st2 = __builtin_fmaf(d, d, st2);
      const float e = __builtin_fabsf(th[b]) - Ka;
      sab1 += e;
      sab2 = __builtin_fmaf(e, e, sab2);
    });
    const float wa = wrapped_step(th[1], th[0]);
    step(wa);
    const float rot = Lanes::next_lane(th[0]);
    if constexpr (!FIRST) {
      const float nxt = Lanes::is_last(lane) ? rot : rot_prev;
      const float wb = wrapped_step(nxt, th_b1_prev);
      step(wb);
      wmax = __builtin_fmaxf(__builtin_fmaxf(wmax, __builtin_fabsf(wa)), __builtin_fabsf(wb));
    } else {
      wmax = __builtin_fabsf(wa);
    }
    if constexpr (LAST) {
      const float w = wrapped_step(rot, th[1]);
      const float wc = Lanes::is_last(lane) ? Kw : w;
      step(wc);
      wmax = __builtin_fmaxf(wmax, __builtin_fabsf(wc));
    }
    th_b1_prev = th[1];
    rot_prev = rot;
  }

  __device__ __forceinline__ void moments(float re0, float im0, float re1, float im1) {
    const float res[2] = {re0, re1}, ims[2] = {im0, im1};
    static_for<2>([&](auto bb) {
      constexpr int b = decltype(bb)::value;
      const float re = res[b], im = ims[b];
      const float q = __builtin_fmaf(im, im, kTinyPower);
      const float P = __builtin_fmaf(re, re, q);
      const float A = __builtin_fmaf(re, re, -q);
      const float Bh = re * im;
      const float AA = A * A, BB = Bh * Bh, AP = A * P;
      const float X4 = __builtin_fmaf(-4.0f, BB, AA);
      sA += A; sBh += Bh; sP += P; sAA += AA; sX4 += X4; sAP += AP;
      sAB = __builtin_fmaf(A, Bh, sAB);
      sBP = __builtin_fmaf(Bh, P, sBP);
      sAAA = __builtin_fmaf(AA, A, sAAA);
      sABB = __builtin_fmaf(A, BB, sABB);
      sAAB = __builtin_fmaf(AA, Bh, sAAB);
      sBBB = __builtin_fmaf(BB, Bh, sBBB);
      sAAP = __builtin_fmaf(AA, P, sAAP);
      sX4P = __builtin_fmaf(X4, P, sX4P);
      sABP = __builtin_fmaf(AP, Bh, sABP);
    });
  }

  __device__ __forceinline__ void clear_sums() {
    sA = sBh = sP = sAA = sX4 = sAB = sAP = sBP = 0.f;
    sAAA = sABB = sAAB = sBBB = sAAP = sX4P = sABP = 0.f;
    sa = st1 = st2 = sab1 = sab2 = sw1 = sw2 = sw3 = sw4 = 0.f;
  }

  __device__ __forceinline__ void envelope(float a, float mu) {
    const float d = a - mu, d2 = d * d;
    sad1 += __builtin_fabsf(d);
    sad2 += d2;
    sad4 = __builtin_fmaf(d2, d2, sad4);
  }
};
using Stats = StatsT<WaveLanes>;


struct LaneAddr {
  const char* tw2;
  const char* tw3;
  char* ex1_w;
  const char* ex1_r;
  char* ex2_w;
  const char* ex2_r;
};

__device__ __forceinline__ void bfly6(float& ar, float& ai, float& br, float& bi, const float2 t) {
  const float yr = __builtin_fmaf(-t.y, bi, __builtin_fmaf(t.x, br, ar));
  const float yi = __builtin_fmaf(t.y, br, __builtin_fmaf(t.x, bi, ai));
  br = __builtin_fmaf(2.0f, ar, -yr);
  bi = __builtin_fmaf(2.0f, ai, -yi);
  ar = yr;
  ai = yi;
}

template <int LEN, class TW>
__device__ __forceinline__ void twisted_dit(float (&re)[LEN], float (&im)[LEN], TW&& tw) {
  constexpr int LOG = LEN == 16 ? 4 : 3;
  static_assert(LEN == 16 || LEN == 8, "pass lengths");
  static_for<LOG>([&](auto ss) {
    constexpr int sidx = decltype(ss)::value;
    constexpr int half = 1 << sidx;
    constexpr int d = LEN / (2 * half);
    static_for<half>([&](auto kk) {
      constexpr int k = decltype(kk)::value;
      const float2 t = tw(std::integral_constant<int, half - 1 + k>{});
      static_for<d>([&](auto mm) {
        constexpr int m = decltype(mm)::value;
        constexpr int p = m + 2 * d * bitrev(k, sidx);
        bfly6(re[p], im[p], re[p + d], im[p + d], t);
      });
    });
  });
}

struct NoFftHook {
  template <class G, class W>
  __device__ __forceinline__ void operator()(G, W) const {}
};

template <int R>
__device__ __forceinline__ void fft_head(const float (&xr)[2 * R], const float (&xi)[2 * R], float (&v0r)[R], float (&v0i)[R],
                                         float (&v1r)[R], float (&v1i)[R]) {
  static_assert(R == 8 || R == 16, "1024 or 2048 points (shorter frames: amcx_short_kernel.h)");
  static_for<R>([&](auto ii) {
    constexpr int i = decltype(ii)::value;
    v0r[i] = xr[2 * i]; v0i[i] = xi[2 * i]; v1r[i] = xr[2 * i + 1]; v1i[i] = xi[2 * i + 1];
  });
  if constexpr (R / 8 == 2) {
    dif_stage<R, 0>(v0r, v0i);
    dif_stage<R, 0>(v1r, v1i);
  }
}

template <int R, bool kDifDone = false, class Hook = NoFftHook>
__device__ __forceinline__ float fft_tail(float (&v0r)[R], float (&v0i)[R], float (&v1r)[R], float (&v1i)[R], const LaneAddr& la,
                                          Hook&& hook = Hook{}) {
  constexpr int PH = R / 8;
  float peak = 0.f;
  static_for<PH>([&](auto gg) {
    constexpr int gph = decltype(gg)::value;
    if constexpr (!kDifDone) {
      dif<8, 8 * gph>(v0r, v0i);
      dif<8, 8 * gph>(v1r, v1i);
    }
    float zr[16], zi[16];
    lds_wave_fence();
    static_for<8>([&](auto kk_) {
      constexpr int kk = decltype(kk_)::value;
      constexpr int p = 8 * gph + bitrev(kk, 3);
      *reinterpret_cast<float2*>(la.ex1_w + (kk * kEx1StrideKK) * 8) = make_float2(v0r[p], v0i[p]);
      *reinterpret_cast<float2*>(la.ex1_w + (kk * kEx1StrideKK + kEx1StrideB) * 8) = make_float2(v1r[p], v1i[p]);
    });
    lds_wave_fence();
    static_for<16>([&](auto nn) {
      constexpr int n2 = decltype(nn)::value;
      const float2 v = *reinterpret_cast<const float2*>(la.ex1_r + n2 * 32);
      zr[n2] = v.x; zi[n2] = v.y;
    });
    hook(gg, std::integral_constant<int, 0>{});
    if constexpr (gph == 0) asm volatile("; MARK fft2");
    if constexpr (gph == 0) __builtin_amdgcn_s_setprio(AMCX_PRIO_OF(4));
    __builtin_amdgcn_sched_barrier(0);
    const char* const tw2 = la.tw2;
    twisted_dit<16>(zr, zi, [&](auto ii) {
      return *reinterpret_cast<const float2*>(tw2 + gph * 8 * kTw2Stride + decltype(ii)::value * 8);
    });
    lds_wave_fence();
    static_for<16>([&](auto kk2) {
      constexpr int k2 = decltype(kk2)::value;
      constexpr int p = bitrev(k2, 4);
      *reinterpret_cast<float2*>(la.ex2_w + (k2 * kEx2StrideK2) * 8) = make_float2(zr[p], zi[p]);
    });
    lds_wave_fence();
    const char* const tw3 = la.tw3;
    static_for<2>([&](auto jj) {
      constexpr int j = decltype(jj)::value;
      float ur[8], ui[8];
      static_for<8>([&](auto nn) {
        constexpr int n3 = decltype(nn)::value;
        const float2 v = *reinterpret_cast<const float2*>(la.ex2_r + (j * 8 * kEx2StrideK2 + n3) * 8);
        ur[n3] = v.x; ui[n3] = v.y;
      });
      if constexpr (j == 0) hook(gg, std::integral_constant<int, 1>{});
      twisted_dit<8>(ur, ui, [&](auto ii) {
        return *reinterpret_cast<const float2*>(tw3 + ((gph * 2 + j) * 7 + decltype(ii)::value) * kTw3Row);
      });
      static_for<4>([&](auto pp) {
        constexpr int p = 2 * decltype(pp)::value;
        peak = __builtin_fmaxf(__builtin_fmaxf(peak, __builtin_fmaf(ur[p], ur[p], ui[p] * ui[p])),
                               __builtin_fmaf(ur[p + 1], ur[p + 1], ui[p + 1] * ui[p + 1]));
      });
    });
    if constexpr (gph + 1 < PH) __builtin_amdgcn_sched_barrier(0);
  });
  lds_wave_fence();
  return peak;
}

template <int R>
__device__ __forceinline__ float fft_peak(const float (&xr)[2 * R], const float (&xi)[2 * R],
                                          const LaneAddr& la) {
  float v0r[R], v0i[R], v1r[R], v1i[R];
  fft_head<R>(xr, xi, v0r, v0i, v1r, v1i);
  return fft_tail<R>(v0r, v0i, v1r, v1i, la);
}

template <int NF>
__device__ __forceinline__ void build_fft_tables(char* t2, char* t3, int tid, int n_threads) {
  constexpr int R = NF / 128, PH = R >= 8 ? R / 8 : 1;
  auto w_nf = [](int e) {
    float sn, cs;
    sincospif((float)(e & (NF - 1)) * (2.0f / (float)NF), &sn, &cs);
    return make_float2(cs, -sn);
  };
  for (int e = tid; e < 8 * PH * 15; e += n_threads) {
    const int slot = e / 15, i = e % 15;
    const int k1 = PH == 2 ? 2 * (slot & 7) + (slot >> 3) : slot % R;
    const int sidx = i < 1 ? 0 : i < 3 ? 1 : i < 7 ? 2 : 3;
    const int k = i - ((1 << sidx) - 1), Lp = 2 << sidx, d = 16 / Lp;
    reinterpret_cast<float2*>(t2)[e] = w_nf(8 * k1 * d + k * (NF / Lp));
  }
  for (int e = tid; e < PH * 2 * 7 * 64; e += n_threads) {
    const int ln = e & 63, i = (e >> 6) % 7, c = e / (7 * 64);
    const int k1 = PH == 2 ? 2 * (ln >> 3) + (c >> 1) : (ln >> 3) % R, k2 = (ln & 7) + 8 * (c & 1);
    const int sidx = i < 1 ? 0 : i < 3 ? 1 : 2;
    const int k = i - ((1 << sidx) - 1), Lp = 2 << sidx, d = 8 / Lp;
    reinterpret_cast<float2*>(t3)[e] = w_nf((R * k2 + k1) * d + k * (NF / Lp));
  }
}

__device__ __forceinline__ double wave_sum_f64(double v) {
#pragma unroll
  for (int off = 32; off >= 1; off >>= 1) v += __shfl_xor(v, off, 64);
  return v;
}

template <int N>
__device__ __forceinline__ void wave_exact_frequency(const float2* __restrict__ src, float sc, float Kw_f, int lane,
                                                     float& f5, float& f9) {
  constexpr int kPer = N / 64, U = kPer < 8 ? kPer : 8, kTrips = kPer / U;
  static_assert(kPer >= 1 && kPer % U == 0, "frame sizes are powers of two >= 128");
  const double Kw = (double)Kw_f;
  double c0 = 0.0, c1 = 0.0, c2 = 0.0, c3 = 0.0;
#pragma unroll 1
  for (int t = 0; t < kTrips; ++t) {
    float2 p[U], q[U];
#pragma unroll
    for (int u = 0; u < U; ++u) {
      const int n = lane + 64 * (U * t + u);
      p[u] = src[n];
      q[u] = src[n + 1 < N ? n + 1 : N - 1];
    }
#pragma unroll
    for (int u = 0; u < U; ++u) {
      const int n = lane + 64 * (U * t + u);
      const float pr = p[u].x * sc, pi = p[u].y * sc, qr = q[u].x * sc, qi = q[u].y * sc;
      const float ap = __builtin_amdgcn_sqrtf(__builtin_fmaf(pr, pr, __builtin_fmaf(pi, pi, kTinyPower)));
      const float aq = __builtin_amdgcn_sqrtf(__builtin_fmaf(qr, qr, __builtin_fmaf(qi, qi, kTinyPower)));
      const float w = exact_step(fast_angle(qr, qi, aq), fast_angle(pr, pi, ap), pr, pi, qr, qi);
      const double d = n < N - 1 ? (double)w - Kw : 0.0, d2 = d * d;
      c0 += d; c1 += d2; c2 += d2 * d; c3 += d2 * d2;
    }
  }
  frequency_features(Kw, wave_sum_f64(c0), wave_sum_f64(c1), wave_sum_f64(c2), wave_sum_f64(c3), N, f5, f9);
}

template <int N>
__device__ __forceinline__ void wave_exact_moments(const float2* __restrict__ src, float sc, int lane, double (&t)[15]) {
  typedef float v4f __attribute__((ext_vector_type(4)));
  typedef const __attribute__((address_space(1))) v4f* gv4f;
  constexpr int kAll = N / 128, kWant = N >= 4096 ? 8 : 4, kG = kAll < kWant ? kAll : kWant, kTrips = kAll / kG;
  static_assert(kAll >= 1 && kAll % kG == 0, "frame sizes are powers of two >= 128");
  gv4f const base = (gv4f)reinterpret_cast<const v4f*>(src + 2 * lane);
  double a[15];
#pragma unroll
  for (int k = 0; k < 15; ++k) a[k] = 0.0;
  v4f nxt[kG];
#pragma unroll
  for (int u = 0; u < kG; ++u) nxt[u] = base[64 * u];
#pragma unroll 1
  for (int tr = 0; tr < kTrips; ++tr) {
    v4f p[kG];
#pragma unroll
    for (int u = 0; u < kG; ++u) p[u] = nxt[u];
    if (tr + 1 < kTrips) {
#pragma unroll
      for (int u = 0; u < kG; ++u) nxt[u] = base[64 * (kG * (tr + 1) + u)];
    }
#pragma unroll
    for (int u = 0; u < 2 * kG; ++u) {
      const double re = (double)(((u & 1) ? p[u >> 1].z : p[u >> 1].x) * sc), im = (double)(((u & 1) ? p[u >> 1].w : p[u >> 1].y) * sc);
      const double im2 = im * im;
      const double A = __builtin_fma(re, re, -im2), P = __builtin_fma(re, re, im2), Bh = re * im;
      const double AA = A * A, BB = Bh * Bh, AP = A * P;
      const double X4 = __builtin_fma(-4.0, BB, AA);
      a[0] += A; a[1] += Bh; a[2] += P; a[3] += AA; a[4] += X4;
      a[5] = __builtin_fma(A, Bh, a[5]);
      a[6] += AP;
      a[7] = __builtin_fma(Bh, P, a[7]);
      a[8] = __builtin_fma(AA, A, a[8]);
      a[9] = __builtin_fma(A, BB, a[9]);
      a[10] = __builtin_fma(AA, Bh, a[10]);
      a[11] = __builtin_fma(BB, Bh, a[11]);
      a[12] = __builtin_fma(AA, P, a[12]);
      a[13] = __builtin_fma(X4, P, a[13]);
      a[14] = __builtin_fma(AP, Bh, a[14]);
      if (u & 1) __builtin_amdgcn_sched_barrier(0);
    }
  }
#pragma unroll 1
  for (int off = 32; off >= 1; off >>= 1) {
#pragma unroll
    for (int k = 0; k < 15; ++k) a[k] += __shfl_xor(a[k], off, 64);
  }
#pragma unroll
  for (int k = 0; k < 15; ++k) t[k] = a[k];
}

template <int N, bool MASKED = false>
__device__ __forceinline__ void wave_exact_cumulants(const float2* __restrict__ src, float sc, int h, int lane, bool mine,
                                                     float* __restrict__ dst_row, unsigned mask = kMaskAll) {
  double t[15];
  wave_exact_moments<N>(src, sc, lane, t);
  if (mine) {
    if constexpr (MASKED) {
      moment_features(t[0], t[1], t[2], t[3], t[4], t[5], t[6], t[7], t[8], t[9], t[10], t[11], t[12], t[13], t[14], (double)N,
                      [&](int j, int twice_order, double v) {
                        if ((mask >> j) & 1u) dst_row[j] = (float)__builtin_ldexp(v, h * twice_order);
                      });
    } else {
      moment_features(t[0], t[1], t[2], t[3], t[4], t[5], t[6], t[7], t[8], t[9], t[10], t[11], t[12], t[13], t[14], (double)N,
                      [&](int j, int twice_order, double v) { dst_row[j] = (float)__builtin_ldexp(v, h * twice_order); });
    }
  }
}

template <int N, int PLAN = kPlanAll>
__device__ __forceinline__ void wave_body(
    const float2* __restrict__ iq, long long n_frames, long long row_stride,
    float* __restrict__ out, long long out_stride, [[maybe_unused]] unsigned mask AMCX_STAMP_ARG) {
  using C = Cfg<N>;
  constexpr int R = C::kFftRows, ROWS = C::kHeldRows;
  constexpr int kWavesPerWG = C::kWavesPerWG, kThreads = C::kThreads, kTailFrames = C::kTailFrames;
  constexpr int kFramesPerWave = C::kFramesPerWave, kTailChunk = C::kTailChunk;
  extern __shared__ float4 amcx_wave_smem[];
  char* smem = reinterpret_cast<char*>(amcx_wave_smem);
  const int tid = threadIdx.x;
  const int lane = tid & 63;
  const int wave = __builtin_amdgcn_readfirstlane(tid >> 6);
  char* t2 = smem;
  char* t3 = smem + C::kT2Bytes;
  char* t4 = smem + C::kTableBytes - C::kT4Bytes;
  char* ex = smem + C::kTableBytes + wave * kExchangeBytes;
  float* stash = reinterpret_cast<float*>(smem + C::kTableBytes + kWavesPerWG * kExchangeBytes) +
                 wave * (kFramesPerWave * C::kFlushes * kStashStride);

  unsigned* const counters = reinterpret_cast<unsigned*>(smem + C::kCounterOffset);
  if (tid == 0) { counters[0] = 0; counters[1] = 0; }
  constexpr int kQ = C::kRunFrames;
  static_assert(kQ % kFramesPerWave == 0 && kFramesPerWave % kTailChunk == 0, "grabs stay inside a run");
  const long long n_wg = gridDim.x, wg = blockIdx.x;
  const long long full_runs = n_frames / kQ;
  const int rem_frames = (int)(n_frames - full_runs * kQ);
  const long long my_full = full_runs > wg ? (full_runs - wg - 1) / n_wg + 1 : 0;
  const long long slice_len = my_full * kQ + (rem_frames > 0 && full_runs % n_wg == wg ? rem_frames : 0);
  const long long body_len = slice_len > kTailFrames ? (slice_len - kTailFrames) / kFramesPerWave * kFramesPerWave : 0;
  const long long tail_len = slice_len - body_len;
  auto frame_of = [&](long long v) -> long long {
    const long long k = v / kQ;
    return (k * n_wg + wg) * kQ + (v - k * kQ);
  };

  if constexpr (PLAN == kPlanAll) {
  build_fft_tables<C::kFftN>(t2, t3, tid, kThreads);
  if constexpr (C::kSplit) {
    for (int e = tid; e < 128; e += kThreads) {
      float sn, cs;
      sincospif((float)e * (1.0f / 2048.0f), &sn, &cs);
      reinterpret_cast<float2*>(t4)[e] = make_float2(cs, -sn);
    }
  }
  }
  __syncthreads();

  const int kkL = lane >> 3, n3L = lane & 7;
  LaneAddr la;
  la.tw2 = t2 + kkL * kTw2Stride;
  la.tw3 = t3 + lane * 8;
  la.ex1_w = ex + lane * 8;
  la.ex1_r = ex + (kkL * kEx1StrideKK + (n3L & 1) * kEx1StrideB + (n3L >> 1)) * 8;
  la.ex2_w = ex + lane * 8;
  la.ex2_r = ex + (n3L * kEx2StrideK2 + kkL * 8) * 8;
  float* const a_lds = reinterpret_cast<float*>(ex) + lane;

#ifdef AMCX_WAVE_STAMPS
  unsigned long long stamp_acc[kStampSections] = {0, 0, 0, 0, 0, 0, 0, 0};
  unsigned long long stamp_last = __builtin_amdgcn_s_memtime();
  const unsigned long long real0 = __builtin_amdgcn_s_memrealtime();
#endif
  for (;;) {
    long long f0;
    int n_here;
    {
      unsigned got = 0;
      if (lane == 0) got = __hip_atomic_fetch_add(&counters[0], (unsigned)kFramesPerWave, __ATOMIC_RELAXED,
                                                  __HIP_MEMORY_SCOPE_WORKGROUP);
      got = __builtin_amdgcn_readfirstlane(got);
      if ((long long)got < body_len) {
        f0 = frame_of(got);
        const long long left = body_len - got;
        n_here = left < kFramesPerWave ? (int)left : kFramesPerWave;
      } else {
        unsigned t = 0;
        if (lane == 0) t = __hip_atomic_fetch_add(&counters[1], (unsigned)kTailChunk, __ATOMIC_RELAXED,
                                                  __HIP_MEMORY_SCOPE_WORKGROUP);
        t = __builtin_amdgcn_readfirstlane(t);
        if ((long long)t >= tail_len) break;
        f0 = frame_of(body_len + t);
        const long long left = tail_len - t;
        n_here = left < kTailChunk ? (int)left : kTailChunk;
      }
    }

    auto load_frame = [&](float (&xr)[2 * ROWS], float (&xi)[2 * ROWS], long long f) {
      const float2* src = iq + f * row_stride + 2 * lane;
      static_for<ROWS>([&](auto ii) {
        constexpr int i = decltype(ii)::value;
        typedef float v4f __attribute__((ext_vector_type(4)));
        const v4f* p = reinterpret_cast<const v4f*>(src + 128 * i);
        const v4f v = __builtin_nontemporal_load(p);
        xr[2 * i] = v.x; xi[2 * i] = v.y; xr[2 * i + 1] = v.z; xi[2 * i + 1] = v.w;
      });
    };
    auto frame = [&](const float (&xr)[2 * ROWS], const float (&xi)[2 * ROWS], int g) {
      asm volatile("; MARK load");
      __builtin_amdgcn_s_setprio(AMCX_PRIO_OF(0));
      AMCX_STAMP(7);
      auto reduce_sums = [&](float (&r28)[28], float (&r7)[7]) __attribute__((always_inline)) {
        asm volatile(
            "s_nop 1\n\t"
            "v_permlane32_swap_b32 %0, %1\n\tv_permlane32_swap_b32 %2, %3\n\t"
            "v_permlane32_swap_b32 %4, %5\n\tv_permlane32_swap_b32 %6, %7\n\t"
            "v_permlane32_swap_b32 %8, %9\n\tv_permlane32_swap_b32 %10, %11\n\t"
            "v_permlane32_swap_b32 %12, %13\n\tv_permlane32_swap_b32 %14, %15\n\t"
            "v_permlane32_swap_b32 %16, %17\n\tv_permlane32_swap_b32 %18, %19\n\t"
            "v_permlane32_swap_b32 %20, %21\n\tv_permlane32_swap_b32 %22, %23\n\t"
            "v_permlane32_swap_b32 %24, %25\n\tv_permlane32_swap_b32 %26, %27"
            : "+v"(r28[0]), "+v"(r28[1]), "+v"(r28[2]), "+v"(r28[3]), "+v"(r28[4]), "+v"(r28[5]),
              "+v"(r28[6]), "+v"(r28[7]), "+v"(r28[8]), "+v"(r28[9]), "+v"(r28[10]), "+v"(r28[11]),
              "+v"(r28[12]), "+v"(r28[13]), "+v"(r28[14]), "+v"(r28[15]), "+v"(r28[16]), "+v"(r28[17]),
              "+v"(r28[18]), "+v"(r28[19]), "+v"(r28[20]), "+v"(r28[21]), "+v"(r28[22]), "+v"(r28[23]),
              "+v"(r28[24]), "+v"(r28[25]), "+v"(r28[26]), "+v"(r28[27]));
        float r14[14];
        static_for<14>([&](auto jj) {
          constexpr int j = decltype(jj)::value;
          r14[j] = r28[2 * j] + r28[2 * j + 1];
        });
        asm volatile(
            "s_nop 1\n\t"
            "v_permlane16_swap_b32 %0, %1\n\tv_permlane16_swap_b32 %2, %3\n\t"
            "v_permlane16_swap_b32 %4, %5\n\tv_permlane16_swap_b32 %6, %7\n\t"
            "v_permlane16_swap_b32 %8, %9\n\tv_permlane16_swap_b32 %10, %11\n\t"
            "v_permlane16_swap_b32 %12, %13"
            : "+v"(r14[0]), "+v"(r14[1]), "+v"(r14[2]), "+v"(r14[3]), "+v"(r14[4]), "+v"(r14[5]),
              "+v"(r14[6]), "+v"(r14[7]), "+v"(r14[8]), "+v"(r14[9]), "+v"(r14[10]), "+v"(r14[11]),
              "+v"(r14[12]), "+v"(r14[13]));
        static_for<7>([&](auto jj) {
          constexpr int j = decltype(jj)::value;
          float v = r14[2 * j] + r14[2 * j + 1];
          v += dpp<kQuadXor1>(v);
          v += dpp<kQuadXor2>(v);
          v += dpp<kRowHalfMirror>(v);
          v += dpp<kRowMirror>(v);
          r7[j] = v;
        });
      };
      auto store_sums = [&](const float (&r7)[7], float* row) __attribute__((always_inline)) {
        int ln = lane;
        asm volatile("" : "+v"(ln));
        if ((ln & 15) == 0) {
          const int rsel = ln >> 4;
          float* dst = row + (((rsel & 1) << 1) | (rsel >> 1));
          static_for<7>([&](auto jj) {
            constexpr int j = decltype(jj)::value;
            dst[4 * j] = r7[j];
          });
        }
      };

      Stats S;
      float sa_flushed = 0.f;
      {
        static_for<ROWS>([&](auto ii) {
          constexpr int i = decltype(ii)::value;
          if constexpr (PLAN == kPlanCumulants) {
            S.moments(xr[2 * i], xi[2 * i], xr[2 * i + 1], xi[2 * i + 1]);
          } else {
          float a0, a1;
          S.template row<i == 0, i == ROWS - 1>(xr[2 * i], xi[2 * i], xr[2 * i + 1], xi[2 * i + 1], lane, a0, a1);
          if constexpr (!C::kSplit) {
            a_lds[(2 * i) * 64] = a0;
            a_lds[(2 * i + 1) * 64] = a1;
          }
          }
          if constexpr (C::kFlushes == 2 && i == ROWS / 2 - 1) {
            __builtin_amdgcn_sched_barrier(0);
            sa_flushed += S.sa;
            float r28[28] = {S.sA, S.sBh, S.sP, S.sAA, S.sX4, S.sAB, S.sAP, S.sBP, S.sAAA, S.sABB,
                             S.sAAB, S.sBBB, S.sAAP, S.sX4P, S.sABP, S.sa, 0.f, 0.f, 0.f,
                             S.st1, S.st2, S.sab1, S.sab2, S.sw1, S.sw2, S.sw3, S.sw4, 0.f};
            float q7[7];
            reduce_sums(r28, q7);
            store_sums(q7, stash + (g * C::kFlushes) * kStashStride);
            S.clear_sums();
            __builtin_amdgcn_sched_barrier(0);
          }
        });
      }
      if constexpr (PLAN != kPlanCumulants) {
      asm volatile("; MARK envelope");
      __builtin_amdgcn_s_setprio(AMCX_PRIO_OF(1));
      AMCX_STAMP(0);
      __builtin_amdgcn_sched_barrier(0);
      const float mu = bcast_l63(wave_sum_l63(S.sa + sa_flushed)) * (1.0f / (float)N);
      {
        static_for<2 * ROWS>([&](auto ee) {
          constexpr int e = decltype(ee)::value;
          if constexpr (C::kSplit) {
            S.envelope(__builtin_amdgcn_sqrtf(__builtin_fmaf(xr[e], xr[e], __builtin_fmaf(xi[e], xi[e], kTinyPower))), mu);
          } else {
            S.envelope(a_lds[e * 64], mu);
          }
        });
      }
      }

      asm volatile("; MARK reduce");
      __builtin_amdgcn_s_setprio(AMCX_PRIO_OF(2));
      AMCX_STAMP(3);
      __builtin_amdgcn_sched_barrier(0);
      float* const row = stash + (g * C::kFlushes + (C::kFlushes - 1)) * kStashStride;
      float r7[7];
      {
        float r28[28] = {S.sA, S.sBh, S.sP, S.sAA, S.sX4, S.sAB, S.sAP, S.sBP, S.sAAA, S.sABB,
                         S.sAAB, S.sBBB, S.sAAP, S.sX4P, S.sABP, S.sa, S.sad1, S.sad2, S.sad4,
                         S.st1, S.st2, S.sab1, S.sab2, S.sw1, S.sw2, S.sw3, S.sw4, 0.f};
        reduce_sums(r28, r7);
      }
      const unsigned long long tie = __builtin_amdgcn_ballot_w64(S.wmax > kPi - kTieBand);
      store_sums(r7, row);
      if (lane == 63) {
        row[kNumSums + 1] = S.Kt;
        row[kNumSums + 2] = S.Kw;
        row[kNumSums + 3] = S.Ka;
        row[kNumSums + 4] = tie != 0 ? 1.0f : 0.0f;
      }

      if constexpr (PLAN == kPlanAll) {
      asm volatile("; MARK fft1");
      AMCX_STAMP(1);
      __builtin_amdgcn_sched_barrier(0);
      __builtin_amdgcn_s_setprio(AMCX_PRIO_OF(3));
      float peak;
      if constexpr (!C::kSplit) {
        peak = fft_peak<R>(xr, xi, la);
      } else {
        auto fft4096 = [&](auto&& row_of) -> float {
          const float4 w4 = *reinterpret_cast<const float4*>(t4 + lane * 16);
          float sr[2 * R], si[2 * R], dr[2 * R], di[2 * R];
          if constexpr (AMCX_PRIO_OF(6) != AMCX_PRIO_OF(3)) __builtin_amdgcn_s_setprio(AMCX_PRIO_OF(6));
          static_for<R>([&](auto ii) {
            constexpr int i = decltype(ii)::value;
            constexpr int lo = 2 * i;
            const float4 p = row_of(std::integral_constant<int, i>{});
            const float4 q = row_of(std::integral_constant<int, R + i>{});
            sr[lo] = p.x + q.x;     si[lo] = p.y + q.y;
            sr[lo + 1] = p.z + q.z; si[lo + 1] = p.w + q.w;
            float d0r = p.x - q.x, d0i = p.y - q.y;
            float d1r = p.z - q.z, d1i = p.w - q.w;
            mul_w32<i>(d0r, d0i);
            mul_w32<i>(d1r, d1i);
            dr[lo] = __builtin_fmaf(d0r, w4.x, -(d0i * w4.y));
            di[lo] = __builtin_fmaf(d0r, w4.y, d0i * w4.x);
            dr[lo + 1] = __builtin_fmaf(d1r, w4.z, -(d1i * w4.w));
            di[lo + 1] = __builtin_fmaf(d1r, w4.w, d1i * w4.z);
          });
          if constexpr (AMCX_PRIO_OF(6) != AMCX_PRIO_OF(3)) {
            __builtin_amdgcn_sched_barrier(0);
            __builtin_amdgcn_s_setprio(AMCX_PRIO_OF(3));
          }
          float s0r[R], s0i[R], s1r[R], s1i[R], d0r[R], d0i[R], d1r[R], d1i[R];
          fft_head<R>(sr, si, s0r, s0i, s1r, s1i);
          const float pk4 = fft_tail<R>(s0r, s0i, s1r, s1i, la, [&](auto gg, auto ww) {
            constexpr int g = decltype(gg)::value, w = decltype(ww)::value;
            if constexpr (g == 0 && w == 0) fft_head<R>(dr, di, d0r, d0i, d1r, d1i);
            if constexpr (g == 0 && w == 1) { dif<8, 0>(d0r, d0i); dif<8, 0>(d1r, d1i); }
            if constexpr (g == 1 && w == 0) { dif<8, 8>(d0r, d0i); dif<8, 8>(d1r, d1i); }
          });
          __builtin_amdgcn_sched_barrier(0);
          return __builtin_fmaxf(pk4, fft_tail<R, true>(d0r, d0i, d1r, d1i, la));
        };
        peak = fft4096([&](auto ic) {
          constexpr int i = decltype(ic)::value;
          return make_float4(xr[2 * i], xi[2 * i], xr[2 * i + 1], xi[2 * i + 1]);
        });
      }

      const float pk = wave_max_l63(peak);
      if (lane == 63) row[kNumSums] = pk;
      }
    };

    auto finalise = [&](auto range_tag, int count) -> unsigned long long {
      constexpr bool RG = decltype(range_tag)::value;
      bool redo = false;
      lds_wave_fence();
      float feat[18];
      long long f = 0;
      [[maybe_unused]] float sc = 1.0f;
      [[maybe_unused]] int ex_half = 0;
      float kw_shift = 0.f;
      bool tie = false, cancel = false;
      [[maybe_unused]] bool flat_angles = true;
      if constexpr (PLAN == kPlanCumulants && !RG) {
        bool tiny = false;
        if (lane < count) {
          const float* row = stash + (lane * C::kFlushes + (C::kFlushes - 1)) * kStashStride;
          double sp = row[2];
          if constexpr (C::kFlushes > 1) {
#pragma unroll
            for (int h = 1; h < C::kFlushes; ++h) sp += (double)row[2 - h * kStashStride];
          }
          tiny = sp <= 2.0 * (double)N * (double)kTinyPower;
        }
        unsigned long long tz = __builtin_amdgcn_ballot_w64(tiny);
        while (tz != 0) {
          const int idx = __builtin_ctzll(tz);
          tz &= tz - 1;
          float xr[2 * ROWS], xi[2 * ROWS];
          load_frame(xr, xi, f0 + idx);
          Stats Z;
          static_for<ROWS>([&](auto ii) {
            constexpr int i = decltype(ii)::value;
            float a0, a1;
            Z.template row<i == 0, i == ROWS - 1>(xr[2 * i], xi[2 * i], xr[2 * i + 1], xi[2 * i + 1], lane, a0, a1);
          });
          const bool flat = __builtin_amdgcn_ballot_w64(Z.st2 != 0.f || Z.sab2 != 0.f) == 0 && Z.Kt == 0.f;
          if (lane == idx) flat_angles = flat;
        }
      }
      if (lane < count) {
        const float* row = stash + (lane * C::kFlushes + (C::kFlushes - 1)) * kStashStride;
        auto sm = [&](int k) -> double {
          double t = row[k];
          if constexpr (C::kFlushes > 1) {
#pragma unroll
            for (int h = 1; h < C::kFlushes; ++h) t += (double)row[k - h * kStashStride];
          }
          return t;
        };
        {
          float s15[15];
#pragma unroll
          for (int k = 0; k < 15; ++k) {
            s15[k] = row[k];
            if constexpr (C::kFlushes > 1) {
#pragma unroll
              for (int h = 1; h < C::kFlushes; ++h) s15[k] += row[k - h * kStashStride];
            }
          }
          cancel = cancellation_suspect(s15, (float)N, (float)cancel_kappa(N));
        }
        FrameSums F;
        F.sA = sm(0); F.sBh = sm(1); F.sP = sm(2); F.sAA = sm(3); F.sX4 = sm(4); F.sAB = sm(5);
        F.sAP = sm(6); F.sBP = sm(7); F.sAAA = sm(8); F.sABB = sm(9); F.sAAB = sm(10);
        F.sBBB = sm(11); F.sAAP = sm(12); F.sX4P = sm(13); F.sABP = sm(14);
        F.sa = sm(15); F.sad1 = sm(16); F.sad2 = sm(17); F.sad4 = sm(18);
        F.std1 = sm(19); F.std2 = sm(20); F.sab1 = sm(21); F.sab2 = sm(22);
        F.swd1 = sm(23); F.swd2 = sm(24); F.swd3 = sm(25); F.swd4 = sm(26);
        F.gmax_raw = row[27]; F.Kt = row[28]; F.Kw = row[29]; F.Ka = row[30];
        F.pi_tie = row[31] != 0.0f;
        kw_shift = row[29];
        if constexpr (PLAN == kPlanCumulants && !RG) {
          if (!flat_angles) F.std2 = 1.0;
        }
        if constexpr (RG) {
          const int code = (int)row[kNumSums + 5];
          const int ex = (code >> 6) - 128;
          cancel = finalize_features<true>(F, N, feat, ex) && cancel;
          sc = __builtin_bit_cast(float, (127 - ex) << 23);
          ex_half = ex / 2;
          f = f0 + (code & 63);
        } else {
          cancel = finalize_features(F, N, feat) && cancel;
          if (is_outside_fp32_range(F, N)) redo = true;
          f = f0 + lane;
        }
        cancel = cancel && !redo;
        tie = __builtin_signbitf(feat[4]) && feat[4] == feat[4] && feat[4] != -__builtin_inff() && !redo;
      }
      if constexpr (PLAN != kPlanAll) {
        if (!(mask & kMaskFreq)) tie = false;
        if (!(mask & kMaskCumulants)) cancel = false;
      }
      unsigned long long ties = __builtin_amdgcn_ballot_w64(tie);
      while (ties != 0) {
        const int idx = __builtin_ctzll(ties);
        ties &= ties - 1;
        const unsigned lo = (unsigned)__builtin_amdgcn_readlane((int)(unsigned)(f & 0xffffffffLL), idx);
        const unsigned hi = (unsigned)__builtin_amdgcn_readlane((int)(unsigned)((unsigned long long)f >> 32), idx);
        const long long ft = (long long)(((unsigned long long)hi << 32) | lo);
        float sct = 1.0f;
        if constexpr (RG) sct = __builtin_bit_cast(float, __builtin_amdgcn_readlane(__builtin_bit_cast(int, sc), idx));
        const float kwt = __builtin_bit_cast(float, __builtin_amdgcn_readlane(__builtin_bit_cast(int, kw_shift), idx));
        float f5x, f9x;
        wave_exact_frequency<N>(iq + ft * row_stride, sct, kwt, lane, f5x, f9x);
        if (lane == idx) { feat[4] = f5x; feat[8] = f9x; }
      }
      if (lane < count && !redo) {
        if constexpr (PLAN != kPlanAll) mask_columns(feat, mask);
        float* dst = out + f * out_stride;
#pragma unroll
        for (int j = 0; j < 18; ++j) dst[j] = feat[j];
      }
      unsigned long long cz = __builtin_amdgcn_ballot_w64(cancel);
      while (cz != 0) {
        const int idx = __builtin_ctzll(cz);
        cz &= cz - 1;
        const unsigned lo = (unsigned)__builtin_amdgcn_readlane((int)(unsigned)(f & 0xffffffffLL), idx);
        const unsigned hi = (unsigned)__builtin_amdgcn_readlane((int)(unsigned)((unsigned long long)f >> 32), idx);
        const long long ft = (long long)(((unsigned long long)hi << 32) | lo);
        float sct = 1.0f;
        int hx = 0;
        if constexpr (RG) {
          sct = __builtin_bit_cast(float, __builtin_amdgcn_readlane(__builtin_bit_cast(int, sc), idx));
          hx = __builtin_amdgcn_readlane(ex_half, idx);
        }
        if constexpr (PLAN == kPlanAll)
          wave_exact_cumulants<N>(iq + ft * row_stride, sct, hx, lane, lane == idx, out + ft * out_stride);
        else
          wave_exact_cumulants<N, true>(iq + ft * row_stride, sct, hx, lane, lane == idx, out + ft * out_stride, mask);
      }
      lds_wave_fence();
      return __builtin_amdgcn_ballot_w64(redo);
    };

    [[maybe_unused]] const LaneAddr& la_redo = la;
    auto rerun_scaled = [&](unsigned long long todo) {
      while (todo != 0) {
        int cnt = 0;
        for (; cnt < kFramesPerWave && todo != 0; ++cnt) {
          const int idx = __builtin_ctzll(todo);
          todo &= todo - 1;
          float xr[2 * ROWS], xi[2 * ROWS];
          load_frame(xr, xi, f0 + idx);
          float m = 0.f;
          static_for<2 * ROWS>([&](auto ee) {
            constexpr int e = decltype(ee)::value;
            m = __builtin_fmaxf(__builtin_fmaxf(m, __builtin_fabsf(xr[e])), __builtin_fabsf(xi[e]));
          });
          m = bcast_l63(wave_max_l63(m));
          int ex = 0;
          if (m >= 0x1p-125f && m <= 3.4028235e38f) ex = (((__builtin_bit_cast(int, m) >> 23) & 0xff) - 127) & ~1;
          const float sc = __builtin_bit_cast(float, (127 - ex) << 23);
          static_for<2 * ROWS>([&](auto ee) {
            constexpr int e = decltype(ee)::value;
            xr[e] *= sc; xi[e] *= sc;
          });
          frame(xr, xi, cnt);
          if (lane == 63)
            stash[(cnt * C::kFlushes + (C::kFlushes - 1)) * kStashStride + kNumSums + 5] = (float)((ex + 128) * 64 + idx);
        }
        finalise(std::true_type{}, cnt);
      }
    };
    for (int g = 0; g < n_here; ++g) {
      float xr[2 * ROWS], xi[2 * ROWS];
      load_frame(xr, xi, f0 + g);
      frame(xr, xi, g);
    }

    AMCX_STAMP(4);
    asm volatile("; MARK finalize");
    __builtin_amdgcn_s_setprio(AMCX_PRIO_OF(5));
    const unsigned long long left_over = finalise(std::false_type{}, n_here);
    asm volatile("; MARK redo");
    if (left_over != 0) rerun_scaled(left_over);
    AMCX_STAMP(5);
  }
#ifdef AMCX_WAVE_STAMPS
  if (lane == 0) {
    const long long w = (long long)blockIdx.x * kWavesPerWG + wave;
    stamp_acc[6] = __builtin_amdgcn_s_memrealtime() - real0;
#if AMCX_WAVE_STAMPS != 1
    stamp_acc[0] = __builtin_amdgcn_s_memtime() - stamp_last;
#endif
    for (int k = 0; k < kStampSections; ++k) stamp_out[w * kStampSections + k] = stamp_acc[k];
  }
#endif
}

template <int N>
__global__ __launch_bounds__(Cfg<N>::kThreads, (Cfg<N>::kWavesPerWG + 3) / 4) void amcx_features18_wave_kernel(
    const float2* __restrict__ iq, long long n_frames, long long row_stride,
    float* __restrict__ out, long long out_stride AMCX_STAMP_ARG) {
#ifdef AMCX_WAVE_STAMPS
  wave_body<N>(iq, n_frames, row_stride, out, out_stride, kMaskAll, stamp_out);
#else
  wave_body<N>(iq, n_frames, row_stride, out, out_stride, kMaskAll);
#endif
}

#ifndef AMCX_WAVE_STAMPS
template <int N, int PLAN>
__global__ __launch_bounds__(Cfg<N>::kThreads, (Cfg<N>::kWavesPerWG + 3) / 4) void amcx_features_subset_wave_kernel(
    const float2* __restrict__ iq, long long n_frames, long long row_stride,
    float* __restrict__ out, long long out_stride, unsigned mask) {
  wave_body<N, PLAN>(iq, n_frames, row_stride, out, out_stride, mask);
}
#endif

}

inline bool wave_supports(int frame_size) {
  return frame_size >= 128 && frame_size <= 32768 && (frame_size & (frame_size - 1)) == 0;
}

inline const char* wave_kernel_name(int frame_size) {
  switch (frame_size) {
    case 128: return "amcx_features18_short_kernel<128>";
    case 256: return "amcx_features18_short_kernel<256>";
    case 512: return "amcx_features18_short_kernel<512>";
    case 1024: return "amcx_features18_wave_kernel<1024>";
    case 2048: return "amcx_features18_wave_kernel<2048>";
    case 4096: return "amcx_features18_wave_kernel<4096>";
    case 8192: return "amcx_features18_quad_kernel";
    case 16384: return "amcx_features18_group_kernel<8>";
    case 32768: return "amcx_features18_group_kernel<16>";
    default: return "";
  }
}

#ifndef AMCX_WAVE_STAMPS
template <int N, int PLAN = kPlanAll>
inline hipError_t launch_wave_n(const float2* iq, int64_t n_frames, int64_t row_stride, float* out,
                                int64_t out_stride, hipStream_t stream, int cus, unsigned mask = kMaskAll) {
  constexpr auto kern = [] {
    if constexpr (PLAN == kPlanAll) return wave::amcx_features18_wave_kernel<N>;
    else return wave::amcx_features_subset_wave_kernel<N, PLAN>;
  }();
  constexpr int lds = wave::Cfg<N>::kLdsBytes;
  static bool lds_attr_set[64] = {};
  int dev = 0;
  hipError_t e = hipGetDevice(&dev);
  if (e != hipSuccess) return e;
  if (dev < 0 || dev >= 64 || !lds_attr_set[dev]) {
    e = hipFuncSetAttribute(reinterpret_cast<const void*>(kern), hipFuncAttributeMaxDynamicSharedMemorySize, lds);
    if (e != hipSuccess) return e;
    if (dev >= 0 && dev < 64) lds_attr_set[dev] = true;
  }
  int64_t grid = (int64_t)cus;
  const int64_t min_slice = wave::Cfg<N>::kWavesPerWG;
  if (grid * min_slice > n_frames) grid = (n_frames + min_slice - 1) / min_slice;
  if constexpr (PLAN == kPlanAll)
    hipLaunchKernelGGL(kern, dim3((unsigned)grid), dim3(wave::Cfg<N>::kThreads), lds, stream, iq,
                       (long long)n_frames, (long long)row_stride, out, (long long)out_stride);
  else
    hipLaunchKernelGGL(kern, dim3((unsigned)grid), dim3(wave::Cfg<N>::kThreads), lds, stream, iq,
                       (long long)n_frames, (long long)row_stride, out, (long long)out_stride, mask);
  return hipGetLastError();
}

template <int PLAN>
inline hipError_t launch_wave_subset(const float2* iq, int64_t n_frames, int32_t frame_size, int64_t row_stride, float* out,
                                     int64_t out_stride, hipStream_t stream, int cus, unsigned mask) {
  switch (frame_size) {
    case 1024: return launch_wave_n<1024, PLAN>(iq, n_frames, row_stride, out, out_stride, stream, cus, mask);
    case 2048: return launch_wave_n<2048, PLAN>(iq, n_frames, row_stride, out, out_stride, stream, cus, mask);
    case 4096: return launch_wave_n<4096, PLAN>(iq, n_frames, row_stride, out, out_stride, stream, cus, mask);
    default: return hipErrorNotSupported;
  }
}

inline hipError_t launch_wave(const float2* iq, int64_t n_frames, int32_t frame_size,
                              int64_t row_stride, float* out, int64_t out_stride,
                              hipStream_t stream, int cus) {
  switch (frame_size) {
    case 1024: return launch_wave_n<1024>(iq, n_frames, row_stride, out, out_stride, stream, cus);
    case 2048: return launch_wave_n<2048>(iq, n_frames, row_stride, out, out_stride, stream, cus);
    case 4096: return launch_wave_n<4096>(iq, n_frames, row_stride, out, out_stride, stream, cus);
    default: return hipErrorNotSupported;
  }
}

#endif

}
```

Baseline: 200.8 million frames/s.

## Batch finaliser over 64 frames via per-wave global ring buffer for N=2048

For 2048-sample frames, each wave now writes its per-frame partial sums to a per-wave ring buffer in global memory instead of the LDS stash, and runs the finaliser once per 64 frames (one frame per lane) rather than once per 4 frames. The amplitude parking also moves into the exchange buffer. The intent is to amortise the lane-underused finaliser step across a full wavefront. The ring is allocated from a per-stream pool or the context, and the old LDS-only kernel is kept as a fallback when no ring is available. The cost is extra global-memory traffic, a host-side mutex and allocation on the launch path, and tail-loop changes so that every wave keeps looping until the batch drains.

```diff
diff --git a/amcpy_amd/csrc/amcx.hip b/amcpy_amd/csrc/amcx.hip
--- a/amcpy_amd/csrc/amcx.hip
+++ b/amcpy_amd/csrc/amcx.hip
@@ -5,7 +5,9 @@
 #include <stdlib.h>
 #include <string.h>
 #include <chrono>
+#include <mutex>
 #include <new>
+#include <vector>
 
 #include "amcx_block_kernel.h"
 #include "amcx_stream_kernel.h"
@@ -60,6 +62,52 @@
   }
   if (dev >= 0 && dev < 64) cus[dev] = n;
   return n;
+}
+
+struct RingSource {
+  float* own = nullptr;
+  size_t own_bytes = 0;
+  bool pool = false;
+};
+struct PoolRing { int device; hipStream_t stream; void* p; size_t bytes; };
+std::mutex g_ring_mu;
+std::vector<PoolRing> g_rings;
+constexpr size_t kPoolRingsPerDevice = 16;
+
+float* pool_ring(hipStream_t stream, size_t bytes) {
+  if (stream == hipStreamPerThread) return nullptr;
+  int dev = 0;
+  if (hipGetDevice(&dev) != hipSuccess) { (void)hipGetLastError(); return nullptr; }
+  hipStreamCaptureStatus cap = hipStreamCaptureStatusNone;
+  if (hipStreamIsCapturing(stream, &cap) != hipSuccess) { (void)hipGetLastError(); return nullptr; }
+  if (cap != hipStreamCaptureStatusNone) return nullptr;
+  std::lock_guard<std::mutex> lock(g_ring_mu);
+  size_t on_dev = 0;
+  for (PoolRing& r : g_rings) {
+    if (r.device != dev) continue;
+    ++on_dev;
+    if (r.stream != stream) continue;
+    if (r.bytes >= bytes) return static_cast<float*>(r.p);
+    (void)hipFree(r.p);
+    r.p = nullptr; r.bytes = 0;
+    if (hipMalloc(&r.p, bytes) != hipSuccess) { (void)hipGetLastError(); r.p = nullptr; return nullptr; }
+    r.bytes = bytes;
+    return static_cast<float*>(r.p);
+  }
+  if (on_dev >= kPoolRingsPerDevice) return nullptr;
+  void* p = nullptr;
+  if (hipMalloc(&p, bytes) != hipSuccess) { (void)hipGetLastError(); return nullptr; }
+  g_rings.push_back(PoolRing{dev, stream, p, bytes});
+  return static_cast<float*>(p);
+}
+
+float* ring_for(const RingSource& rs, int32_t N, hipStream_t stream) {
+  static const bool off = [] { const char* t = getenv("AMCX_WAVE_RING"); return t != nullptr && t[0] == '0'; }();
+  if (off) return nullptr;
+  const size_t need = amcx::wave_ring_bytes(N, cu_count());
+  if (need == 0) return nullptr;
+  if (rs.own != nullptr) return rs.own_bytes >= need ? rs.own : nullptr;
+  return rs.pool ? pool_ring(stream, need) : nullptr;
 }
 
 bool on_another_device(const void* p) {
@@ -228,6 +276,11 @@
   if (threadIdx.x == 0) partial[blockIdx.x] = (s[0] + s[1]) + (s[2] + s[3]);
 }
 
+
+int features18_ws(const void* iq_dev, int64_t n_frames, int32_t frame_size, int64_t row_stride_elems, float* out_dev,
+                  int64_t out_row_stride, void* hip_stream, int32_t variant, void* workspace_dev, int64_t workspace_bytes,
+                  const RingSource& rings);
+
 }
 
 extern "C" {
@@ -274,6 +327,19 @@
 int amcx_features18_c64_ws(const void* iq_dev, int64_t n_frames, int32_t frame_size,
                            int64_t row_stride_elems, float* out_dev, int64_t out_row_stride,
                            void* hip_stream, int32_t variant, void* workspace_dev, int64_t workspace_bytes) {
+  RingSource rings;
+  rings.pool = true;
+  return features18_ws(iq_dev, n_frames, frame_size, row_stride_elems, out_dev, out_row_stride, hip_stream, variant,
+                       workspace_dev, workspace_bytes, rings);
+}
+
+}
+
+namespace {
+
+int features18_ws(const void* iq_dev, int64_t n_frames, int32_t frame_size, int64_t row_stride_elems, float* out_dev,
+                  int64_t out_row_stride, void* hip_stream, int32_t variant, void* workspace_dev, int64_t workspace_bytes,
+                  const RingSource& rings) {
   if (n_frames < 0 || row_stride_elems < frame_size || out_row_stride < AMCX_NUM_FEATURES)
     return AMCX_EINVAL;
   const int v = resolve_variant(frame_size, variant);
@@ -296,7 +362,8 @@
     else if (amcx::shortk::short_supports(frame_size))
       e = amcx::shortk::launch_short(iq, n_frames, frame_size, row_stride_elems, out_dev, out_row_stride, stream, cu_count());
     else
-      e = amcx::launch_wave(iq, n_frames, frame_size, row_stride_elems, out_dev, out_row_stride, stream, cu_count());
+      e = amcx::launch_wave(iq, n_frames, frame_size, row_stride_elems, out_dev, out_row_stride, stream, cu_count(),
+                            ring_for(rings, frame_size, stream));
     if (e != hipSuccess) return hip_fail(e, "wave kernel launch");
     return AMCX_OK;
   }
@@ -304,6 +371,10 @@
   return launch_block(iq, n_frames, frame_size, row_stride_elems, out_dev, out_row_stride, stream, workspace_dev,
                       workspace_bytes < 0 ? 0 : workspace_bytes);
 }
+
+}
+
+extern "C" {
 
 int amcx_features18_c64_ex(const void* iq_dev, int64_t n_frames, int32_t frame_size,
                            int64_t row_stride_elems, float* out_dev, int64_t out_row_stride,
@@ -358,13 +429,9 @@
   return (mask & ~amcx::kMaskCumulants) == 0 ? amcx::kPlanCumulants : amcx::kPlanNoSpectral;
 }
 
-}
-
-extern "C" {
-
-int amcx_features_c64_subset(const void* iq_dev, int64_t n_frames, int32_t frame_size, int64_t row_stride_elems,
-                             float* out_dev, int64_t out_row_stride, void* hip_stream, int32_t variant, uint32_t feature_mask,
-                             void* workspace_dev, int64_t workspace_bytes) {
+int features_subset(const void* iq_dev, int64_t n_frames, int32_t frame_size, int64_t row_stride_elems,
+                    float* out_dev, int64_t out_row_stride, void* hip_stream, int32_t variant, uint32_t feature_mask,
+                    void* workspace_dev, int64_t workspace_bytes, const RingSource& rings) {
   if (!valid_feature_mask(feature_mask)) return AMCX_EINVAL;
   if (n_frames < 0 || row_stride_elems < frame_size || out_row_stride < AMCX_NUM_FEATURES) return AMCX_EINVAL;
   const int v = resolve_variant(frame_size, variant);
@@ -374,8 +441,8 @@
   hipStream_t stream = static_cast<hipStream_t>(hip_stream);
   const int plan = subset_plan(frame_size, v, feature_mask);
   if (plan == amcx::kPlanAll) {
-    const int rc = amcx_features18_c64_ws(iq_dev, n_frames, frame_size, row_stride_elems, out_dev, out_row_stride,
-                                          hip_stream, variant, workspace_dev, workspace_bytes);
+    const int rc = features18_ws(iq_dev, n_frames, frame_size, row_stride_elems, out_dev, out_row_stride,
+                                 hip_stream, variant, workspace_dev, workspace_bytes, rings);
     if (rc != AMCX_OK || feature_mask == (uint32_t)AMCX_FEATURES_ALL) return rc;
     int64_t grid = (n_frames * AMCX_NUM_FEATURES + 255) / 256;
     if (grid > 8192) grid = 8192;
@@ -388,19 +455,33 @@
   if (on_another_device(iq_dev) || on_another_device(out_dev)) return AMCX_EINVAL;
   const float2* iq = static_cast<const float2*>(iq_dev);
   const bool short_n = amcx::shortk::short_supports(frame_size);
+  float* const ring = short_n ? nullptr : ring_for(rings, frame_size, stream);
   hipError_t e;
   if (plan == amcx::kPlanCumulants)
     e = short_n ? amcx::shortk::launch_short_subset<amcx::kPlanCumulants>(iq, n_frames, frame_size, row_stride_elems, out_dev,
                                                                          out_row_stride, stream, cu_count(), feature_mask)
                 : amcx::launch_wave_subset<amcx::kPlanCumulants>(iq, n_frames, frame_size, row_stride_elems, out_dev,
-                                                                 out_row_stride, stream, cu_count(), feature_mask);
+                                                                 out_row_stride, stream, cu_count(), ring, feature_mask);
   else
     e = short_n ? amcx::shortk::launch_short_subset<amcx::kPlanNoSpectral>(iq, n_frames, frame_size, row_stride_elems, out_dev,
                                                                           out_row_stride, stream, cu_count(), feature_mask)
                 : amcx::launch_wave_subset<amcx::kPlanNoSpectral>(iq, n_frames, frame_size, row_stride_elems, out_dev,
-                                                                  out_row_stride, stream, cu_count(), feature_mask);
+                                                                  out_row_stride, stream, cu_count(), ring, feature_mask);
   if (e != hipSuccess) return hip_fail(e, "feature-subset kernel launch");
   return AMCX_OK;
+}
+
+}
+
+extern "C" {
+
+int amcx_features_c64_subset(const void* iq_dev, int64_t n_frames, int32_t frame_size, int64_t row_stride_elems,
+                             float* out_dev, int64_t out_row_stride, void* hip_stream, int32_t variant, uint32_t feature_mask,
+                             void* workspace_dev, int64_t workspace_bytes) {
+  RingSource rings;
+  rings.pool = true;
+  return features_subset(iq_dev, n_frames, frame_size, row_stride_elems, out_dev, out_row_stride, hip_stream, variant,
+                         feature_mask, workspace_dev, workspace_bytes, rings);
 }
 
 struct amcx_ctx {
@@ -416,6 +497,7 @@
   void* d_slab = nullptr;  size_t slab_cap = 0;
   void* d_frames = nullptr; size_t frames_cap = 0;
   void* d_ws = nullptr; size_t ws_cap = 0;
+  void* d_ring = nullptr; size_t ring_cap = 0;
   hipEvent_t up_done[3] = {nullptr, nullptr, nullptr};
   hipEvent_t slab_free[2] = {nullptr, nullptr};
   float* out_pin = nullptr; size_t out_pin_cap = 0;
@@ -459,16 +541,21 @@
 void ctx_reserve_ws(amcx_ctx* c, int32_t N, int64_t frames, int32_t variant) {
   const int64_t want = amcx_features18_workspace_bytes(N, frames, variant);
   if (want > 0 && ctx_reserve(&c->d_ws, &c->ws_cap, (size_t)want) != AMCX_OK) { c->d_ws = nullptr; c->ws_cap = 0; }
+  const size_t ring = resolve_variant(N, variant) == AMCX_VARIANT_WAVE ? amcx::wave_ring_bytes(N, cu_count()) : 0;
+  if (ring > 0 && ctx_reserve(&c->d_ring, &c->ring_cap, ring) != AMCX_OK) { c->d_ring = nullptr; c->ring_cap = 0; }
 }
 
 int ctx_features(amcx_ctx* c, const void* rows, int64_t frames, int32_t N, float* out, int32_t variant, uint32_t mask) {
   const int64_t want = amcx_features18_workspace_bytes(N, frames, variant);
   const bool have = want > 0 && c->d_ws != nullptr && c->ws_cap >= (size_t)want;
+  RingSource rings;
+  rings.own = static_cast<float*>(c->d_ring);
+  rings.own_bytes = c->ring_cap;
   if (mask != (uint32_t)AMCX_FEATURES_ALL)
-    return amcx_features_c64_subset(rows, frames, N, N, out, AMCX_NUM_FEATURES, c->stream, variant, mask,
-                                    have ? c->d_ws : nullptr, have ? want : 0);
-  return amcx_features18_c64_ws(rows, frames, N, N, out, AMCX_NUM_FEATURES, c->stream, variant, have ? c->d_ws : nullptr,
-                                have ? want : 0);
+    return features_subset(rows, frames, N, N, out, AMCX_NUM_FEATURES, c->stream, variant, mask,
+                           have ? c->d_ws : nullptr, have ? want : 0, rings);
+  return features18_ws(rows, frames, N, N, out, AMCX_NUM_FEATURES, c->stream, variant, have ? c->d_ws : nullptr,
+                       have ? want : 0, rings);
 }
 
 struct DeviceGuard {
@@ -890,6 +977,7 @@
   if (c->d_slab) (void)hipFree(c->d_slab);
   if (c->d_frames) (void)hipFree(c->d_frames);
   if (c->d_ws) (void)hipFree(c->d_ws);
+  if (c->d_ring) (void)hipFree(c->d_ring);
   if (c->pin) (void)hipHostFree(c->pin);
   if (c->out_pin) (void)hipHostFree(c->out_pin);
   for (auto& g : c->graphs) if (g.exec) (void)hipGraphExecDestroy(g.exec);
diff --git a/amcpy_amd/csrc/amcx_wave_kernel.h b/amcpy_amd/csrc/amcx_wave_kernel.h
--- a/amcpy_amd/csrc/amcx_wave_kernel.h
+++ b/amcpy_amd/csrc/amcx_wave_kernel.h
@@ -39,6 +39,9 @@
   static constexpr int kFramesPerWave = N == 2048 ? 4 : 8;
   static constexpr int kFlushes = N == 4096 ? 2 : 1;
   static constexpr int kStashBytes = kFramesPerWave * kFlushes * kStashStride * 4;
+  static constexpr int kFinaliseFrames = N == 2048 ? 64 : kFramesPerWave;
+  static constexpr bool kHasRing = kFinaliseFrames > kFramesPerWave;
+  static constexpr int kRingFloatsPerWave = kFinaliseFrames * kFlushes * kStashStride;
   static constexpr int kTailChunk = 2;
   static constexpr int kRunFrames = kFramesPerWave;
   static constexpr int kWavesPerWG = kSplit ? 8 : 16;
@@ -56,7 +59,8 @@
   static constexpr int kCounterOffset = kTableBytes + kWavesPerWG * (kExchangeBytes + kStashBytes);
   static constexpr int kLdsBytes = kCounterOffset + 16;
   static_assert(kLdsBytes <= 163840, "one workgroup per CU must fit in 160 KiB of LDS");
-  static_assert(kFramesPerWave <= 64, "one frame per lane in the finaliser");
+  static_assert(kFramesPerWave <= 64 && kFinaliseFrames <= 64, "one frame per lane in the finaliser");
+  static_assert(kFinaliseFrames % kFramesPerWave == 0, "a batch is whole runs");
   static_assert(kSplit || 2 * kRows * 64 * 4 <= kExchangeBytes, "|x| parking must fit the exchange buffer");
 };
 
@@ -605,11 +609,12 @@
   }
 }
 
-template <int N, int PLAN = kPlanAll>
+template <int N, int PLAN = kPlanAll, bool RING = Cfg<N>::kHasRing>
 __device__ __forceinline__ void wave_body(
     const float2* __restrict__ iq, long long n_frames, long long row_stride,
-    float* __restrict__ out, long long out_stride, [[maybe_unused]] unsigned mask AMCX_STAMP_ARG) {
+    float* __restrict__ out, long long out_stride, [[maybe_unused]] unsigned mask, [[maybe_unused]] float* ring AMCX_STAMP_ARG) {
   using C = Cfg<N>;
+  static_assert(!RING || C::kHasRing, "no ring form at this frame size");
   constexpr int R = C::kFftRows, ROWS = C::kHeldRows;
   constexpr int kWavesPerWG = C::kWavesPerWG, kThreads = C::kThreads, kTailFrames = C::kTailFrames;
   constexpr int kFramesPerWave = C::kFramesPerWave, kTailChunk = C::kTailChunk;
@@ -624,6 +629,11 @@
   char* ex = smem + C::kTableBytes + wave * kExchangeBytes;
   float* stash = reinterpret_cast<float*>(smem + C::kTableBytes + kWavesPerWG * kExchangeBytes) +
                  wave * (kFramesPerWave * C::kFlushes * kStashStride);
+  constexpr int kBatch = RING ? C::kFinaliseFrames : kFramesPerWave;
+  [[maybe_unused]] float* ring_w = nullptr;
+  if constexpr (RING) ring_w = ring + ((long long)blockIdx.x * kWavesPerWG + wave) * (long long)C::kRingFloatsPerWave;
+  [[maybe_unused]] int filled = 0;
+  [[maybe_unused]] long long batch_f = 0;
 
   unsigned* const counters = reinterpret_cast<unsigned*>(smem + C::kCounterOffset);
   if (tid == 0) { counters[0] = 0; counters[1] = 0; }
@@ -685,10 +695,19 @@
         if (lane == 0) t = __hip_atomic_fetch_add(&counters[1], (unsigned)kTailChunk, __ATOMIC_RELAXED,
                                                   __HIP_MEMORY_SCOPE_WORKGROUP);
         t = __builtin_amdgcn_readfirstlane(t);
-        if ((long long)t >= tail_len) break;
-        f0 = frame_of(body_len + t);
-        const long long left = tail_len - t;
-        n_here = left < kTailChunk ? (int)left : kTailChunk;
+        if constexpr (!RING) {
+          if ((long long)t >= tail_len) break;
+          f0 = frame_of(body_len + t);
+          const long long left = tail_len - t;
+          n_here = left < kTailChunk ? (int)left : kTailChunk;
+        } else if ((long long)t >= tail_len) {
+          f0 = 0;
+          n_here = 0;
+        } else {
+          f0 = frame_of(body_len + t);
+          const long long left = tail_len - t;
+          n_here = left < kTailChunk ? (int)left : kTailChunk;
+        }
       }
     }
 
@@ -702,7 +721,22 @@
         xr[2 * i] = v.x; xi[2 * i] = v.y; xr[2 * i + 1] = v.z; xi[2 * i + 1] = v.w;
       });
     };
-    auto frame = [&](const float (&xr)[2 * ROWS], const float (&xi)[2 * ROWS], int g) {
+    auto frame = [&](const float (&xr)[2 * ROWS], const float (&xi)[2 * ROWS], int g, [[maybe_unused]] long long fidx,
+                     auto to_ring) {
+      constexpr bool TO_RING = decltype(to_ring)::value;
+      float* const rows = [&]() -> float* {
+        if constexpr (TO_RING) return ring_w;
+        else return stash;
+      }();
+      float* const a_park = [&]() -> float* {
+        if constexpr (RING) {
+          int ln = lane;
+          asm volatile("" : "+v"(ln));
+          return reinterpret_cast<float*>(ex) + ln;
+        } else {
+          return a_lds;
+        }
+      }();
       asm volatile("; MARK load");
       __builtin_amdgcn_s_setprio(AMCX_PRIO_OF(0));
       AMCX_STAMP(7);
@@ -769,8 +803,8 @@
           float a0, a1;
           S.template row<i == 0, i == ROWS - 1>(xr[2 * i], xi[2 * i], xr[2 * i + 1], xi[2 * i + 1], lane, a0, a1);
           if constexpr (!C::kSplit) {
-            a_lds[(2 * i) * 64] = a0;
-            a_lds[(2 * i + 1) * 64] = a1;
+            a_park[(2 * i) * 64] = a0;
+            a_park[(2 * i + 1) * 64] = a1;
           }
           }
           if constexpr (C::kFlushes == 2 && i == ROWS / 2 - 1) {
@@ -781,7 +815,7 @@
                              S.st1, S.st2, S.sab1, S.sab2, S.sw1, S.sw2, S.sw3, S.sw4, 0.f};
             float q7[7];
             reduce_sums(r28, q7);
-            store_sums(q7, stash + (g * C::kFlushes) * kStashStride);
+            store_sums(q7, rows + (g * C::kFlushes) * kStashStride);
             S.clear_sums();
             __builtin_amdgcn_sched_barrier(0);
           }
@@ -799,7 +833,7 @@
           if constexpr (C::kSplit) {
             S.envelope(__builtin_amdgcn_sqrtf(__builtin_fmaf(xr[e], xr[e], __builtin_fmaf(xi[e], xi[e], kTinyPower))), mu);
           } else {
-            S.envelope(a_lds[e * 64], mu);
+            S.envelope(a_park[e * 64], mu);
           }
         });
       }
@@ -809,7 +843,7 @@
       __builtin_amdgcn_s_setprio(AMCX_PRIO_OF(2));
       AMCX_STAMP(3);
       __builtin_amdgcn_sched_barrier(0);
-      float* const row = stash + (g * C::kFlushes + (C::kFlushes - 1)) * kStashStride;
+      float* const row = rows + (g * C::kFlushes + (C::kFlushes - 1)) * kStashStride;
       float r7[7];
       {
         float r28[28] = {S.sA, S.sBh, S.sP, S.sAA, S.sX4, S.sAB, S.sAP, S.sBP, S.sAAA, S.sABB,
@@ -823,7 +857,13 @@
         row[kNumSums + 1] = S.Kt;
         row[kNumSums + 2] = S.Kw;
         row[kNumSums + 3] = S.Ka;
-        row[kNumSums + 4] = tie != 0 ? 1.0f : 0.0f;
+        if constexpr (TO_RING) {
+          const unsigned long long fu = (unsigned long long)fidx;
+          row[kNumSums + 4] = __builtin_bit_cast(float, ((unsigned)(fu >> 32) << 1) | (tie != 0 ? 1u : 0u));
+          row[kNumSums + 5] = __builtin_bit_cast(float, (unsigned)fu);
+        } else {
+          row[kNumSums + 4] = tie != 0 ? 1.0f : 0.0f;
+        }
       }
 
       if constexpr (PLAN == kPlanAll) {
@@ -883,10 +923,42 @@
 
     auto finalise = [&](auto range_tag, int count) -> unsigned long long {
       constexpr bool RG = decltype(range_tag)::value;
+      constexpr bool FROM_RING = RING && !RG;
       bool redo = false;
       lds_wave_fence();
+      auto lane_row = [&]() -> const float* {
+        if constexpr (RING) {
+          int ln = lane;
+          asm volatile("" : "+v"(ln));
+          if constexpr (FROM_RING) return ring_w + (ln * C::kFlushes + (C::kFlushes - 1)) * kStashStride;
+          else return stash + (ln * C::kFlushes + (C::kFlushes - 1)) * kStashStride;
+        } else {
+          return stash + (lane * C::kFlushes + (C::kFlushes - 1)) * kStashStride;
+        }
+      };
       float feat[18];
       long long f = 0;
+      if constexpr (FROM_RING) {
+        __builtin_amdgcn_fence(__ATOMIC_RELEASE, "workgroup");
+        __builtin_amdgcn_fence(__ATOMIC_ACQUIRE, "workgroup");
+        if (lane < count) {
+          const float* row = lane_row();
+          const unsigned hi_tie = __builtin_bit_cast(unsigned, row[kNumSums + 4]);
+          f = (long long)(((unsigned long long)(hi_tie >> 1) << 32) | __builtin_bit_cast(unsigned, row[kNumSums + 5]));
+        }
+      }
+      [[maybe_unused]] auto frame_of_lane = [&](long long fl, int idx) -> long long {
+        const unsigned lo = (unsigned)__builtin_amdgcn_readlane((int)(unsigned)(fl & 0xffffffffLL), idx);
+        const unsigned hi = (unsigned)__builtin_amdgcn_readlane((int)(unsigned)((unsigned long long)fl >> 32), idx);
+        return (long long)(((unsigned long long)hi << 32) | lo);
+      };
+      if constexpr (RG && RING) {
+        int src = 0;
+        if (lane < count) src = (int)lane_row()[kNumSums + 5] & 63;
+        const unsigned lo = (unsigned)__builtin_amdgcn_ds_bpermute(src * 4, (int)(unsigned)(batch_f & 0xffffffffLL));
+        const unsigned hi = (unsigned)__builtin_amdgcn_ds_bpermute(src * 4, (int)(unsigned)((unsigned long long)batch_f >> 32));
+        f = (long long)(((unsigned long long)hi << 32) | lo);
+      }
       [[maybe_unused]] float sc = 1.0f;
       [[maybe_unused]] int ex_half = 0;
       float kw_shift = 0.f;
@@ -895,7 +967,7 @@
       if constexpr (PLAN == kPlanCumulants && !RG) {
         bool tiny = false;
         if (lane < count) {
-          const float* row = stash + (lane * C::kFlushes + (C::kFlushes - 1)) * kStashStride;
+          const float* row = lane_row();
           double sp = row[2];
           if constexpr (C::kFlushes > 1) {
 #pragma unroll
@@ -908,7 +980,8 @@
           const int idx = __builtin_ctzll(tz);
           tz &= tz - 1;
           float xr[2 * ROWS], xi[2 * ROWS];
-          load_frame(xr, xi, f0 + idx);
+          if constexpr (RING) load_frame(xr, xi, frame_of_lane(f, idx));
+          else load_frame(xr, xi, f0 + idx);
           Stats Z;
           static_for<ROWS>([&](auto ii) {
             constexpr int i = decltype(ii)::value;
@@ -920,12 +993,23 @@
         }
       }
       if (lane < count) {
-        const float* row = stash + (lane * C::kFlushes + (C::kFlushes - 1)) * kStashStride;
+        const float* row = lane_row();
+        [[maybe_unused]] float rb[FROM_RING ? C::kFlushes * kStashStride : 1];
+        if constexpr (FROM_RING) {
+#pragma unroll
+          for (int h = 0; h < C::kFlushes; ++h)
+#pragma unroll
+            for (int k = 0; k < kStashStride; ++k) rb[h * kStashStride + k] = row[k - h * kStashStride];
+        }
+        auto rd = [&](int k, int h) -> float {
+          if constexpr (FROM_RING) return rb[h * kStashStride + k];
+          else return row[k - h * kStashStride];
+        };
         auto sm = [&](int k) -> double {
-          double t = row[k];
+          double t = rd(k, 0);
           if constexpr (C::kFlushes > 1) {
 #pragma unroll
-            for (int h = 1; h < C::kFlushes; ++h) t += (double)row[k - h * kStashStride];
+            for (int h = 1; h < C::kFlushes; ++h) t += (double)rd(k, h);
           }
           return t;
         };
@@ -933,10 +1017,10 @@
           float s15[15];
 #pragma unroll
           for (int k = 0; k < 15; ++k) {
-            s15[k] = row[k];
+            s15[k] = rd(k, 0);
             if constexpr (C::kFlushes > 1) {
 #pragma unroll
-              for (int h = 1; h < C::kFlushes; ++h) s15[k] += row[k - h * kStashStride];
+              for (int h = 1; h < C::kFlushes; ++h) s15[k] += rd(k, h);
             }
           }
           cancel = cancellation_suspect(s15, (float)N, (float)cancel_kappa(N));
@@ -948,9 +1032,10 @@
         F.sa = sm(15); F.sad1 = sm(16); F.sad2 = sm(17); F.sad4 = sm(18);
         F.std1 = sm(19); F.std2 = sm(20); F.sab1 = sm(21); F.sab2 = sm(22);
         F.swd1 = sm(23); F.swd2 = sm(24); F.swd3 = sm(25); F.swd4 = sm(26);
-        F.gmax_raw = row[27]; F.Kt = row[28]; F.Kw = row[29]; F.Ka = row[30];
-        F.pi_tie = row[31] != 0.0f;
-        kw_shift = row[29];
+        F.gmax_raw = rd(27, 0); F.Kt = rd(28, 0); F.Kw = rd(29, 0); F.Ka = rd(30, 0);
+        if constexpr (FROM_RING) F.pi_tie = (__builtin_bit_cast(unsigned, rd(31, 0)) & 1u) != 0;
+        else F.pi_tie = rd(31, 0) != 0.0f;
+        kw_shift = rd(29, 0);
         if constexpr (PLAN == kPlanCumulants && !RG) {
           if (!flat_angles) F.std2 = 1.0;
         }
@@ -960,11 +1045,11 @@
           cancel = finalize_features<true>(F, N, feat, ex) && cancel;
           sc = __builtin_bit_cast(float, (127 - ex) << 23);
           ex_half = ex / 2;
-          f = f0 + (code & 63);
+          if constexpr (!RING) f = f0 + (code & 63);
         } else {
           cancel = finalize_features(F, N, feat) && cancel;
           if (is_outside_fp32_range(F, N)) redo = true;
-          f = f0 + lane;
+          if constexpr (!RING) f = f0 + lane;
         }
         cancel = cancel && !redo;
         tie = __builtin_signbitf(feat[4]) && feat[4] == feat[4] && feat[4] != -__builtin_inff() && !redo;
@@ -1012,6 +1097,7 @@
           wave_exact_cumulants<N, true>(iq + ft * row_stride, sct, hx, lane, lane == idx, out + ft * out_stride, mask);
       }
       lds_wave_fence();
+      if constexpr (FROM_RING) batch_f = f;
       return __builtin_amdgcn_ballot_w64(redo);
     };
 
@@ -1023,7 +1109,13 @@
           const int idx = __builtin_ctzll(todo);
           todo &= todo - 1;
           float xr[2 * ROWS], xi[2 * ROWS];
-          load_frame(xr, xi, f0 + idx);
+          if constexpr (RING) {
+            const unsigned lo = (unsigned)__builtin_amdgcn_readlane((int)(unsigned)(batch_f & 0xffffffffLL), idx);
+            const unsigned hi = (unsigned)__builtin_amdgcn_readlane((int)(unsigned)((unsigned long long)batch_f >> 32), idx);
+            load_frame(xr, xi, (long long)(((unsigned long long)hi << 32) | lo));
+          } else {
+            load_frame(xr, xi, f0 + idx);
+          }
           float m = 0.f;
           static_for<2 * ROWS>([&](auto ee) {
             constexpr int e = decltype(ee)::value;
@@ -1037,7 +1129,7 @@
             constexpr int e = decltype(ee)::value;
             xr[e] *= sc; xi[e] *= sc;
           });
-          frame(xr, xi, cnt);
+          frame(xr, xi, cnt, 0, std::false_type{});
           if (lane == 63)
             stash[(cnt * C::kFlushes + (C::kFlushes - 1)) * kStashStride + kNumSums + 5] = (float)((ex + 128) * 64 + idx);
         }
@@ -1047,16 +1139,28 @@
     for (int g = 0; g < n_here; ++g) {
       float xr[2 * ROWS], xi[2 * ROWS];
       load_frame(xr, xi, f0 + g);
-      frame(xr, xi, g);
+      if constexpr (RING) frame(xr, xi, filled + g, f0 + g, std::true_type{});
+      else frame(xr, xi, g, 0, std::false_type{});
+    }
+    [[maybe_unused]] int batch = n_here;
+    if constexpr (RING) {
+      filled += n_here;
+      if (n_here != 0 && filled + kFramesPerWave <= kBatch) continue;
+      if (filled == 0) break;
+      batch = filled;
     }
 
     AMCX_STAMP(4);
     asm volatile("; MARK finalize");
     __builtin_amdgcn_s_setprio(AMCX_PRIO_OF(5));
-    const unsigned long long left_over = finalise(std::false_type{}, n_here);
+    const unsigned long long left_over = finalise(std::false_type{}, batch);
     asm volatile("; MARK redo");
     if (left_over != 0) rerun_scaled(left_over);
     AMCX_STAMP(5);
+    if constexpr (RING) {
+      filled = 0;
+      if (n_here == 0) break;
+    }
   }
 #ifdef AMCX_WAVE_STAMPS
   if (lane == 0) {
@@ -1070,23 +1174,57 @@
 #endif
 }
 
+#ifdef AMCX_WAVE_STAMPS
 template <int N>
 __global__ __launch_bounds__(Cfg<N>::kThreads, (Cfg<N>::kWavesPerWG + 3) / 4) void amcx_features18_wave_kernel(
     const float2* __restrict__ iq, long long n_frames, long long row_stride,
-    float* __restrict__ out, long long out_stride AMCX_STAMP_ARG) {
-#ifdef AMCX_WAVE_STAMPS
-  wave_body<N>(iq, n_frames, row_stride, out, out_stride, kMaskAll, stamp_out);
+    float* __restrict__ out, long long out_stride, float* ring AMCX_STAMP_ARG) {
+  wave_body<N>(iq, n_frames, row_stride, out, out_stride, kMaskAll, ring, stamp_out);
+}
 #else
-  wave_body<N>(iq, n_frames, row_stride, out, out_stride, kMaskAll);
+template <int N>
+__global__ __launch_bounds__(Cfg<N>::kThreads, (Cfg<N>::kWavesPerWG + 3) / 4) void amcx_features18_wave_kernel(
+    const float2* __restrict__ iq, long long n_frames, long long row_stride,
+    float* __restrict__ out, long long out_stride) {
+  static_assert(!Cfg<N>::kHasRing, "this size's kernel takes a ring; its LDS form is amcx_features18_wave_lds_kernel");
+  wave_body<N, kPlanAll, false>(iq, n_frames, row_stride, out, out_stride, kMaskAll, nullptr);
+}
+template <int N>
+__global__ __launch_bounds__(Cfg<N>::kThreads, (Cfg<N>::kWavesPerWG + 3) / 4) void amcx_features18_wave_kernel(
+    const float2* __restrict__ iq, long long n_frames, long long row_stride,
+    float* __restrict__ out, long long out_stride, float* ring) {
+  static_assert(Cfg<N>::kHasRing, "no ring form at this frame size");
+  wave_body<N, kPlanAll, true>(iq, n_frames, row_stride, out, out_stride, kMaskAll, ring);
+}
 #endif
-}
 
 #ifndef AMCX_WAVE_STAMPS
 template <int N, int PLAN>
 __global__ __launch_bounds__(Cfg<N>::kThreads, (Cfg<N>::kWavesPerWG + 3) / 4) void amcx_features_subset_wave_kernel(
     const float2* __restrict__ iq, long long n_frames, long long row_stride,
     float* __restrict__ out, long long out_stride, unsigned mask) {
-  wave_body<N, PLAN>(iq, n_frames, row_stride, out, out_stride, mask);
+  static_assert(!Cfg<N>::kHasRing, "this size's kernel takes a ring; its LDS form is amcx_features_subset_wave_lds_kernel");
+  wave_body<N, PLAN, false>(iq, n_frames, row_stride, out, out_stride, mask, nullptr);
+}
+template <int N, int PLAN>
+__global__ __launch_bounds__(Cfg<N>::kThreads, (Cfg<N>::kWavesPerWG + 3) / 4) void amcx_features_subset_wave_kernel(
+    const float2* __restrict__ iq, long long n_frames, long long row_stride,
+    float* __restrict__ out, long long out_stride, unsigned mask, float* ring) {
+  static_assert(Cfg<N>::kHasRing, "no ring form at this frame size");
+  wave_body<N, PLAN, true>(iq, n_frames, row_stride, out, out_stride, mask, ring);
+}
+
+template <int N>
+__global__ __launch_bounds__(Cfg<N>::kThreads, (Cfg<N>::kWavesPerWG + 3) / 4) void amcx_features18_wave_lds_kernel(
+    const float2* __restrict__ iq, long long n_frames, long long row_stride,
+    float* __restrict__ out, long long out_stride) {
+  wave_body<N, kPlanAll, false>(iq, n_frames, row_stride, out, out_stride, kMaskAll, nullptr);
+}
+template <int N, int PLAN>
+__global__ __launch_bounds__(Cfg<N>::kThreads, (Cfg<N>::kWavesPerWG + 3) / 4) void amcx_features_subset_wave_lds_kernel(
+    const float2* __restrict__ iq, long long n_frames, long long row_stride,
+    float* __restrict__ out, long long out_stride, unsigned mask) {
+  wave_body<N, PLAN, false>(iq, n_frames, row_stride, out, out_stride, mask, nullptr);
 }
 #endif
 
@@ -1112,53 +1250,112 @@
 }
 
 #ifndef AMCX_WAVE_STAMPS
-template <int N, int PLAN = kPlanAll>
-inline hipError_t launch_wave_n(const float2* iq, int64_t n_frames, int64_t row_stride, float* out,
-                                int64_t out_stride, hipStream_t stream, int cus, unsigned mask = kMaskAll) {
-  constexpr auto kern = [] {
-    if constexpr (PLAN == kPlanAll) return wave::amcx_features18_wave_kernel<N>;
-    else return wave::amcx_features_subset_wave_kernel<N, PLAN>;
-  }();
-  constexpr int lds = wave::Cfg<N>::kLdsBytes;
-  static bool lds_attr_set[64] = {};
+inline size_t wave_ring_bytes(int frame_size, int cus) {
+  auto of = [&](auto cfg) -> size_t {
+    using C = decltype(cfg);
+    return C::kHasRing ? (size_t)cus * C::kWavesPerWG * C::kRingFloatsPerWave * sizeof(float) : 0;
+  };
+  switch (frame_size) {
+    case 1024: return of(wave::Cfg<1024>{});
+    case 2048: return of(wave::Cfg<2048>{});
+    case 4096: return of(wave::Cfg<4096>{});
+    default: return 0;
+  }
+}
+
+template <class K>
+inline hipError_t wave_lds_attr(K kern, int lds, bool (&set)[64]) {
   int dev = 0;
   hipError_t e = hipGetDevice(&dev);
   if (e != hipSuccess) return e;
-  if (dev < 0 || dev >= 64 || !lds_attr_set[dev]) {
+  if (dev < 0 || dev >= 64 || !set[dev]) {
     e = hipFuncSetAttribute(reinterpret_cast<const void*>(kern), hipFuncAttributeMaxDynamicSharedMemorySize, lds);
     if (e != hipSuccess) return e;
-    if (dev >= 0 && dev < 64) lds_attr_set[dev] = true;
-  }
+    if (dev >= 0 && dev < 64) set[dev] = true;
+  }
+  return hipSuccess;
+}
+
+template <int N, int PLAN = kPlanAll>
+inline hipError_t launch_wave_n(const float2* iq, int64_t n_frames, int64_t row_stride, float* out,
+                                int64_t out_stride, hipStream_t stream, int cus, float* ring, unsigned mask = kMaskAll) {
+  using Plain18 = void (*)(const float2*, long long, long long, float*, long long);
+  using Ring18 = void (*)(const float2*, long long, long long, float*, long long, float*);
+  using PlainSub = void (*)(const float2*, long long, long long, float*, long long, unsigned);
+  using RingSub = void (*)(const float2*, long long, long long, float*, long long, unsigned, float*);
+  constexpr bool kRing = wave::Cfg<N>::kHasRing;
+  constexpr auto kern = [] {
+    if constexpr (PLAN == kPlanAll) {
+      if constexpr (kRing) return static_cast<Ring18>(wave::amcx_features18_wave_kernel<N>);
+      else return static_cast<Plain18>(wave::amcx_features18_wave_kernel<N>);
+    } else {
+      if constexpr (kRing) return static_cast<RingSub>(wave::amcx_features_subset_wave_kernel<N, PLAN>);
+      else return static_cast<PlainSub>(wave::amcx_features_subset_wave_kernel<N, PLAN>);
+    }
+  }();
+  constexpr int lds = wave::Cfg<N>::kLdsBytes;
+  const bool lds_form = wave::Cfg<N>::kHasRing && ring == nullptr;
+  static bool lds_attr_set[64] = {};
+  hipError_t e = hipSuccess;
+  if (!lds_form) e = wave_lds_attr(kern, lds, lds_attr_set);
+  if (e != hipSuccess) return e;
   int64_t grid = (int64_t)cus;
   const int64_t min_slice = wave::Cfg<N>::kWavesPerWG;
   if (grid * min_slice > n_frames) grid = (n_frames + min_slice - 1) / min_slice;
-  if constexpr (PLAN == kPlanAll)
-    hipLaunchKernelGGL(kern, dim3((unsigned)grid), dim3(wave::Cfg<N>::kThreads), lds, stream, iq,
-                       (long long)n_frames, (long long)row_stride, out, (long long)out_stride);
-  else
-    hipLaunchKernelGGL(kern, dim3((unsigned)grid), dim3(wave::Cfg<N>::kThreads), lds, stream, iq,
-                       (long long)n_frames, (long long)row_stride, out, (long long)out_stride, mask);
+  if constexpr (wave::Cfg<N>::kHasRing) {
+    if (lds_form) {
+      constexpr auto kern_lds = [] {
+        if constexpr (PLAN == kPlanAll) return wave::amcx_features18_wave_lds_kernel<N>;
+        else return wave::amcx_features_subset_wave_lds_kernel<N, PLAN>;
+      }();
+      static bool lds_attr_set_lds[64] = {};
+      e = wave_lds_attr(kern_lds, lds, lds_attr_set_lds);
+      if (e != hipSuccess) return e;
+      if constexpr (PLAN == kPlanAll)
+        hipLaunchKernelGGL(kern_lds, dim3((unsigned)grid), dim3(wave::Cfg<N>::kThreads), lds, stream, iq,
+                           (long long)n_frames, (long long)row_stride, out, (long long)out_stride);
+      else
+        hipLaunchKernelGGL(kern_lds, dim3((unsigned)grid), dim3(wave::Cfg<N>::kThreads), lds, stream, iq,
+                           (long long)n_frames, (long long)row_stride, out, (long long)out_stride, mask);
+      return hipGetLastError();
+    }
+  }
+  if constexpr (kRing) {
+    if constexpr (PLAN == kPlanAll)
+      hipLaunchKernelGGL(kern, dim3((unsigned)grid), dim3(wave::Cfg<N>::kThreads), lds, stream, iq,
+                         (long long)n_frames, (long long)row_stride, out, (long long)out_stride, ring);
+    else
+      hipLaunchKernelGGL(kern, dim3((unsigned)grid), dim3(wave::Cfg<N>::kThreads), lds, stream, iq,
+                         (long long)n_frames, (long long)row_stride, out, (long long)out_stride, mask, ring);
+  } else {
+    if constexpr (PLAN == kPlanAll)
+      hipLaunchKernelGGL(kern, dim3((unsigned)grid), dim3(wave::Cfg<N>::kThreads), lds, stream, iq,
+                         (long long)n_frames, (long long)row_stride, out, (long long)out_stride);
+    else
+      hipLaunchKernelGGL(kern, dim3((unsigned)grid), dim3(wave::Cfg<N>::kThreads), lds, stream, iq,
+                         (long long)n_frames, (long long)row_stride, out, (long long)out_stride, mask);
+  }
   return hipGetLastError();
 }
 
 template <int PLAN>
 inline hipError_t launch_wave_subset(const float2* iq, int64_t n_frames, int32_t frame_size, int64_t row_stride, float* out,
-                                     int64_t out_stride, hipStream_t stream, int cus, unsigned mask) {
+                                     int64_t out_stride, hipStream_t stream, int cus, float* ring, unsigned mask) {
   switch (frame_size) {
-    case 1024: return launch_wave_n<1024, PLAN>(iq, n_frames, row_stride, out, out_stride, stream, cus, mask);
-    case 2048: return launch_wave_n<2048, PLAN>(iq, n_frames, row_stride, out, out_stride, stream, cus, mask);
-    case 4096: return launch_wave_n<4096, PLAN>(iq, n_frames, row_stride, out, out_stride, stream, cus, mask);
+    case 1024: return launch_wave_n<1024, PLAN>(iq, n_frames, row_stride, out, out_stride, stream, cus, ring, mask);
+    case 2048: return launch_wave_n<2048, PLAN>(iq, n_frames, row_stride, out, out_stride, stream, cus, ring, mask);
+    case 4096: return launch_wave_n<4096, PLAN>(iq, n_frames, row_stride, out, out_stride, stream, cus, ring, mask);
     default: return hipErrorNotSupported;
   }
 }
 
 inline hipError_t launch_wave(const float2* iq, int64_t n_frames, int32_t frame_size,
                               int64_t row_stride, float* out, int64_t out_stride,
-                              hipStream_t stream, int cus) {
+                              hipStream_t stream, int cus, float* ring) {
   switch (frame_size) {
-    case 1024: return launch_wave_n<1024>(iq, n_frames, row_stride, out, out_stride, stream, cus);
-    case 2048: return launch_wave_n<2048>(iq, n_frames, row_stride, out, out_stride, stream, cus);
-    case 4096: return launch_wave_n<4096>(iq, n_frames, row_stride, out, out_stride, stream, cus);
+    case 1024: return launch_wave_n<1024>(iq, n_frames, row_stride, out, out_stride, stream, cus, ring);
+    case 2048: return launch_wave_n<2048>(iq, n_frames, row_stride, out, out_stride, stream, cus, ring);
+    case 4096: return launch_wave_n<4096>(iq, n_frames, row_stride, out, out_stride, stream, cus, ring);
     default: return hipErrorNotSupported;
   }
 }
```

New measurement: 206.3 million frames/s, median of 6. 1.03x the previous value.
